# JiuTongBro/MultiView_Inpaint

Hardware: AMD Instinct MI355X
Metric: Mpix/s fwd+bwd @1.5M Gauss 1080p (higher is better)
Workload: dtype f32; 1 GPU; rasterizer-with-depth fwd+bwd, one 1920x1080 view per GPU per step, N=1500000 Gaussians, sh_degree 3 (BASELINE.json configs[2] size, SURVEY.md §8d scene); gaussians=1500000, visible=1312313, num_rendered_D=14779663, tiles=8160, tile_list_max=2266, parallelism=views x1

## Files before the change

### include/mvi_raster.h

```cpp
#ifndef MVI_RASTER_H
#define MVI_RASTER_H

#include <stddef.h>
#include <stdint.h>

#ifdef __cplusplus
extern "C" {
#endif

#define MVI_OK 0
#define MVI_EINVAL (-1)
#define MVI_EHIP (-2)
#define MVI_ENOMEM (-3)

#define MVI_TILE 16

typedef struct mvi_raster_settings {
    int32_t image_height;
    int32_t image_width;
    float tanfovx;
    float tanfovy;
    float scale_modifier;
    int32_t sh_degree;
    int32_t prefiltered;
    const float* bg;
    const float* viewmatrix;
    const float* projmatrix;
    const float* campos;
} mvi_raster_settings;

size_t mvi_raster_geom_bytes(int32_t P);
size_t mvi_raster_image_bytes(int32_t image_width, int32_t image_height);
size_t mvi_raster_binning_bytes(int64_t num_rendered, int32_t image_width, int32_t image_height);

int mvi_raster_forward_geom(const mvi_raster_settings* s, int32_t P, int32_t M,
                            const float* means3D, const float* shs, const float* colors_precomp,
                            const float* opacities, const float* scales, const float* rotations,
                            const float* cov3D_precomp, void* geom, size_t geom_bytes,
                            int32_t* radii, int64_t* num_rendered_host, void* stream);

int mvi_raster_forward_render(const mvi_raster_settings* s, int32_t P, int64_t num_rendered,
                              const int32_t* radii, void* geom, size_t geom_bytes, void* binning, size_t binning_bytes,
                              void* image, size_t image_bytes, float* out_color, float* out_depth,
                              void* stream);
int mvi_raster_forward_render_prepare(const mvi_raster_settings* s, int32_t P, int64_t num_rendered,
                                      const int32_t* radii, void* geom, size_t geom_bytes, void* binning,
                                      size_t binning_bytes, void* image, size_t image_bytes, float* out_color,
                                      float* out_depth, float* grad_rows_scratch, void* stream);

int mvi_raster_backward(const mvi_raster_settings* s, int32_t P, int32_t M, int64_t num_rendered,
                        const float* means3D, const float* shs, const float* colors_precomp,
                        const float* scales, const float* rotations, const float* cov3D_precomp,
                        const int32_t* radii, const void* geom, const void* binning,
                        const void* image, const float* dL_dout_color, float* dL_dmeans3D,
                        float* dL_dmeans2D, float* dL_dopacity, float* dL_dshs, float* dL_dcolors,
                        float* dL_dscales, float* dL_drotations, float* dL_dcov3D,
                        float* grad_rows_scratch, int32_t grad_rows_prezeroed, void* stream);

int mvi_raster_forward_geom_raw(const mvi_raster_settings* s, int32_t P, int32_t M, const float* xyz,
                                const float* features_dc, const float* features_rest, const float* raw_opacity,
                                const float* raw_scaling, const float* raw_rotation, void* geom, size_t geom_bytes,
                                int32_t* radii, int64_t* num_rendered_host, void* stream);
int mvi_raster_backward_raw(const mvi_raster_settings* s, int32_t P, int32_t M, int64_t num_rendered, const float* xyz,
                            const float* features_dc, const float* features_rest, const float* raw_opacity,
                            const float* raw_scaling, const float* raw_rotation, const int32_t* radii, const void* geom,
                            const void* binning, const void* image, const float* dL_dout_color, float* dL_dxyz,
                            float* dL_dmeans2D, float* dL_draw_opacity, float* dL_dfeatures_dc, float* dL_dfeatures_rest,
                            float* dL_draw_scaling, float* dL_draw_rotation, float* grad_rows_scratch, 
                            int32_t grad_rows_prezeroed, void* stream);
int mvi_raster_backward_raw_factor(const mvi_raster_settings* s, int32_t P, int32_t M, int64_t num_rendered, const float* xyz,
                                   const float* features_dc, const float* features_rest, const float* raw_opacity,
                                   const float* raw_scaling, const float* raw_rotation, const int32_t* radii, const void* geom,
                                   const void* binning, const void* image, const float* dL_dout_color, float* dL_dxyz,
                                   float* dL_dmeans2D, float* dL_draw_opacity, float* dL_dsh_color_factor,
                                   float* dL_draw_scaling, float* dL_draw_rotation, float* grad_rows_scratch,
                                   int32_t grad_rows_prezeroed, void* stream);

int mvi_raster_sh_backward_views(int32_t P, int32_t M, int32_t sh_degree, int32_t n_views, const float* means3D,
                                 const float* campos, int64_t campos_stride, const float* dL_dcolors,
                                 int64_t colors_view_stride, float* dL_dshs, void* stream);

int mvi_raster_mark_visible(int32_t P, const float* means3D, const float* viewmatrix,
                            const float* projmatrix, uint8_t* visible, void* stream);

int mvi_raster_backward_render(const mvi_raster_settings* s, int32_t P, int64_t num_rendered, const int32_t* radii,
                               const void* geom, const void* binning, const void* image, const float* dL_dout_color,
                               float* grad_rows_scratch, float* dL_dcolor_factor, int32_t sh_input,
                               int32_t grad_rows_prezeroed, void* stream);
int mvi_raster_backward_geom(const mvi_raster_settings* s, int32_t P, int32_t M, const float* means3D, const float* shs,
                             const float* colors_precomp, const float* scales, const float* rotations,
                             const float* cov3D_precomp, const int32_t* radii, const void* geom,
                             const float* grad_rows_scratch, float* dL_dmeans3D, float* dL_dmeans2D, float* dL_dopacity,
                             float* dL_dshs, float* dL_dcolors, float* dL_dscales, float* dL_drotations, float* dL_dcov3D,
                             void* stream);

int mvi_raster_backward_geom_range(const mvi_raster_settings* s, int32_t P, int32_t M, int32_t first, int32_t count,
                                   const float* means3D, const float* shs, const float* colors_precomp, const float* scales,
                                   const float* rotations, const float* cov3D_precomp, const int32_t* radii, const void* geom,
                                   const float* grad_rows_scratch, float* dL_dmeans3D, float* dL_dmeans2D, float* dL_dopacity,
                                   float* dL_dshs, float* dL_dcolors, float* dL_dscales, float* dL_drotations, float* dL_dcov3D,
                                   void* stream);

typedef struct mvi_raster_views {
    const float* depths;
    const float* means2D;
    const float* cov3D_a;
    const float* cov3D_b;
    const float* conic_opacity;
    const float* rgbd;
    const uint32_t* tiles_touched;
    const uint8_t* clamped;
    const void* tile_ids_sorted;
    const uint32_t* point_list;
    const uint32_t* ranges;
    const float* final_T;
    const uint32_t* n_contrib;
    int32_t tile_id_bytes;
    const uint8_t* grad_support;
} mvi_raster_views;
int mvi_raster_get_views(int32_t P, int64_t num_rendered, int32_t image_width, int32_t image_height,
                         const void* geom, const void* binning, const void* image,
                         mvi_raster_views* out);

#define MVI_RASTER_NSTAGES 8
int mvi_raster_timing_enable(int enable);
int mvi_raster_timing_enable_stages(uint32_t stage_mask);
int mvi_raster_timing_read(float* ms_sum_host, int32_t* calls_host);
const char* mvi_raster_stage_name(int stage);

int mvi_raster_color_mode(int deferred);
int mvi_raster_resolve_colors(const mvi_raster_settings* s, int32_t P, void* geom, size_t geom_bytes, void* stream);

int mvi_raster_binning_version(int version);
int mvi_raster_backward_mode(int dense);
int mvi_raster_dev_stamps(int pass, void* device_buffer);

const char* mvi_raster_last_error(void);
const char* mvi_version(void);

#ifdef __cplusplus
}
#endif
#endif
```

### multiview_inpaint_amd/_lib.py

```python
import ctypes as C
import os
import re

_HERE = os.path.dirname(os.path.abspath(__file__))
LIB_PATH = os.environ.get("MVI_HIP_LIB") or os.path.join(_HERE, "csrc", "libmvi_hip.so")
LIB_OVERRIDDEN = bool(os.environ.get("MVI_HIP_LIB"))
if LIB_OVERRIDDEN:
    import sys as _sys
    _sys.stderr.write(f"[mvi] MVI_HIP_LIB is set: every kernel comes from {LIB_PATH}, not from the in-tree build\n")
INCLUDE_DIR = os.path.normpath(os.path.join(_HERE, "..", "include"))


class RasterSettings(C.Structure):
    _fields_ = [
        ("image_height", C.c_int32), ("image_width", C.c_int32),
        ("tanfovx", C.c_float), ("tanfovy", C.c_float), ("scale_modifier", C.c_float),
        ("sh_degree", C.c_int32), ("prefiltered", C.c_int32),
        ("bg", C.c_void_p), ("viewmatrix", C.c_void_p), ("projmatrix", C.c_void_p), ("campos", C.c_void_p),
    ]


class RasterViews(C.Structure):
    _fields_ = [(n, C.c_void_p) for n in (
        "depths", "means2D", "cov3D_a", "cov3D_b", "conic_opacity", "rgbd", "tiles_touched", "clamped",
        "tile_ids_sorted", "point_list", "ranges", "final_T", "n_contrib")] + [("tile_id_bytes", C.c_int32),
                                                                                   ("grad_support", C.c_void_p)]


class AdamGroup(C.Structure):
    _fields_ = [("param", C.c_void_p), ("grad", C.c_void_p), ("exp_avg", C.c_void_p), ("exp_avg_sq", C.c_void_p),
                ("n", C.c_int64), ("lr", C.c_float)]


class CompactTensor(C.Structure):
    _fields_ = [("in_", C.c_void_p), ("out", C.c_void_p), ("width", C.c_int32), ("packed_stride", C.c_int32)]


def declared_symbols():
    names = []
    for fn in sorted(os.listdir(INCLUDE_DIR)):
        if fn.endswith(".h"):
            src = open(os.path.join(INCLUDE_DIR, fn)).read()
            src = re.sub(r"/\*.*?\*/", "", src, flags=re.S)
            names += re.findall(r"\b(mvi_[a-z0-9_]+)\s*\(", src)
    return sorted(set(names))


def raster_source_digest():
    import hashlib
    h = hashlib.sha1()
    d = os.path.join(_HERE, "csrc")
    for fn in sorted(os.listdir(d)):
        if fn.startswith("raster_") and fn.endswith((".hip", ".h")):
            h.update(fn.encode())
            h.update(open(os.path.join(d, fn), "rb").read())
    return h.hexdigest()[:16]


_lib = None


def lib():
    global _lib
    if _lib is not None:
        return _lib
    if not os.path.exists(LIB_PATH):
        raise RuntimeError(
            f"{LIB_PATH} is missing: the HIP extension is not built. Run `python -m multiview_inpaint_amd.build` "
            "(hipcc --offload-arch=gfx950). There is no CPU or PyTorch fallback for this path.")
    L = C.CDLL(LIB_PATH)
    missing = [s for s in declared_symbols() if not hasattr(L, s)]
    if missing:
        raise RuntimeError(f"{LIB_PATH} does not export {missing}; rebuild it")
    vp, i32, i64, sz = C.c_void_p, C.c_int32, C.c_int64, C.c_size_t
    L.mvi_raster_last_error.restype = C.c_char_p
    L.mvi_version.restype = C.c_char_p
    L.mvi_raster_geom_bytes.restype = sz
    L.mvi_raster_geom_bytes.argtypes = [i32]
    L.mvi_raster_image_bytes.restype = sz
    L.mvi_raster_image_bytes.argtypes = [i32, i32]
    L.mvi_raster_binning_bytes.restype = sz
    L.mvi_raster_binning_bytes.argtypes = [i64, i32, i32]
    L.mvi_raster_forward_geom.restype = C.c_int
    L.mvi_raster_forward_geom.argtypes = [C.POINTER(RasterSettings), i32, i32] + [vp] * 7 + [vp, sz, vp, C.POINTER(i64), vp]
    L.mvi_raster_forward_render.restype = C.c_int
    L.mvi_raster_forward_render.argtypes = [C.POINTER(RasterSettings), i32, i64, vp, vp, sz, vp, sz, vp, sz, vp, vp, vp]
    L.mvi_raster_forward_render_prepare.restype = C.c_int
    L.mvi_raster_forward_render_prepare.argtypes = [C.POINTER(RasterSettings), i32, i64, vp, vp, sz, vp, sz, vp, sz, vp, vp, vp, vp]
    L.mvi_raster_backward.restype = C.c_int
    L.mvi_raster_backward.argtypes = [C.POINTER(RasterSettings), i32, i32, i64] + [vp] * 20 + [i32, vp]
    L.mvi_raster_backward_render.restype = C.c_int
    L.mvi_raster_backward_render.argtypes = [C.POINTER(RasterSettings), i32, i64] + [vp] * 7 + [i32, i32, vp]
    L.mvi_raster_backward_geom.restype = C.c_int
    L.mvi_raster_backward_geom.argtypes = [C.POINTER(RasterSettings), i32, i32] + [vp] * 18
    L.mvi_raster_backward_geom_range.restype = C.c_int
    L.mvi_raster_backward_geom_range.argtypes = [C.POINTER(RasterSettings), i32, i32, i32, i32] + [vp] * 18
    L.mvi_raster_forward_geom_raw.restype = C.c_int
    L.mvi_raster_forward_geom_raw.argtypes = [C.POINTER(RasterSettings), i32, i32] + [vp] * 6 + [vp, sz, vp, C.POINTER(i64), vp]
    L.mvi_raster_backward_raw.restype = C.c_int
    L.mvi_raster_backward_raw.argtypes = [C.POINTER(RasterSettings), i32, i32, i64] + [vp] * 19 + [i32, vp]
    L.mvi_raster_backward_raw_factor.restype = C.c_int
    L.mvi_raster_backward_raw_factor.argtypes = [C.POINTER(RasterSettings), i32, i32, i64] + [vp] * 18 + [i32, vp]
    L.mvi_raster_sh_backward_views.restype = C.c_int
    L.mvi_raster_sh_backward_views.argtypes = [i32, i32, i32, i32, vp, vp, i64, vp, i64, vp, vp]
    L.mvi_raster_mark_visible.restype = C.c_int
    L.mvi_raster_mark_visible.argtypes = [i32, vp, vp, vp, vp, vp]
    L.mvi_raster_get_views.restype = C.c_int
    L.mvi_raster_get_views.argtypes = [i32, i64, i32, i32, vp, vp, vp, C.POINTER(RasterViews)]
    L.mvi_raster_timing_enable.restype = C.c_int
    L.mvi_raster_timing_enable.argtypes = [C.c_int]
    L.mvi_raster_timing_enable_stages.restype = C.c_int
    L.mvi_raster_timing_enable_stages.argtypes = [C.c_uint32]
    L.mvi_raster_timing_read.restype = C.c_int
    L.mvi_raster_timing_read.argtypes = [C.POINTER(C.c_float), C.POINTER(C.c_int32)]
    L.mvi_raster_stage_name.restype = C.c_char_p
    L.mvi_raster_stage_name.argtypes = [C.c_int]
    L.mvi_raster_binning_version.restype = C.c_int
    L.mvi_raster_binning_version.argtypes = [C.c_int]
    L.mvi_raster_backward_mode.restype = C.c_int
    L.mvi_raster_backward_mode.argtypes = [C.c_int]
    L.mvi_raster_color_mode.restype = C.c_int
    L.mvi_raster_color_mode.argtypes = [C.c_int]
    L.mvi_raster_resolve_colors.restype = C.c_int
    L.mvi_raster_resolve_colors.argtypes = [C.POINTER(RasterSettings), i32, vp, sz, vp]
    L.mvi_raster_dev_stamps.restype = C.c_int
    L.mvi_raster_dev_stamps.argtypes = [C.c_int, vp]
    _bind_unet_ops(L)
    _bind_train_ops(L)
    _bind_box_region(L)
    _lib = L
    return L


def _bind_unet_ops(L):
    try:
        from . import _unet_ops_bind
    except ImportError:
        return
    _unet_ops_bind.bind(L)


def _bind_train_ops(L):
    vp, i32, sz, f32 = C.c_void_p, C.c_int32, C.c_size_t, C.c_float
    L.mvi_photometric_loss_workspace_bytes.restype = sz
    L.mvi_photometric_loss_workspace_bytes.argtypes = [i32, i32]
    L.mvi_photometric_loss.restype = C.c_int
    L.mvi_photometric_loss.argtypes = [vp, vp, vp, i32, i32, f32, f32, vp, vp, vp, sz, vp]
    L.mvi_photometric_loss_stats.restype = C.c_int
    L.mvi_photometric_loss_stats.argtypes = [vp, vp, vp, i32, i32, vp, vp, sz, vp]
    L.mvi_photometric_loss_grad2.restype = C.c_int
    L.mvi_photometric_loss_grad2.argtypes = [vp, vp, vp, i32, i32, vp, vp, vp, sz, vp]
    L.mvi_train_last_error.restype = C.c_char_p
    L.mvi_knn3_mean_dist2.restype = C.c_int
    L.mvi_knn3_mean_dist2.argtypes = [vp, i32, vp, vp]
    L.mvi_adam_step.restype = C.c_int
    L.mvi_adam_step.argtypes = [C.POINTER(AdamGroup), i32, C.c_double, C.c_double, C.c_double, i32, vp]
    L.mvi_compact_workspace_bytes.restype = sz
    L.mvi_compact_workspace_bytes.argtypes = [i32]
    L.mvi_compact_plan.restype = C.c_int
    L.mvi_compact_plan.argtypes = [vp, i32, vp, sz, vp, vp]
    L.mvi_compact_gather.restype = C.c_int
    L.mvi_compact_gather.argtypes = [C.POINTER(CompactTensor), i32, i32, C.c_uint32, vp, vp]
    L.mvi_support_pack_bits.restype = C.c_int
    L.mvi_support_pack_bits.argtypes = [vp, i32, vp, vp]
    L.mvi_support_union_bits.restype = C.c_int
    L.mvi_support_union_bits.argtypes = [vp, i32, i32, vp, vp]
    for f in (L.mvi_compact_gather_window, L.mvi_compact_scatter_window):
        f.restype = C.c_int
        f.argtypes = [C.POINTER(CompactTensor), i32, i32, vp, C.c_uint32, C.c_uint32, vp, vp]
    L.mvi_gaussian_activations.restype = C.c_int
    L.mvi_gaussian_activations.argtypes = [i32, i32] + [vp] * 10
    L.mvi_gaussian_activations_backward.restype = C.c_int
    L.mvi_gaussian_activations_backward.argtypes = [i32, i32] + [vp] * 13


def _bind_box_region(L):
    vp, i32, i64 = C.c_void_p, C.c_int32, C.c_int64
    L.mvi_box_region_last_error.restype = C.c_char_p
    L.mvi_mesh_intersect.restype = C.c_int
    L.mvi_mesh_intersect.argtypes = [vp, vp, i64, vp, i32, vp, vp, vp, vp, vp]
    L.mvi_mesh_points_inside.restype = C.c_int
    L.mvi_mesh_points_inside.argtypes = [vp, i64, vp, i32, vp, vp]
    L.mvi_mesh_view_masks.restype = C.c_int
    L.mvi_mesh_view_masks.argtypes = [vp, vp, vp, i32, i32, i32, vp, i32, vp, vp, vp, vp, vp, vp]


def check(rc, what):
    if rc != 0:
        msg = lib().mvi_raster_last_error().decode(errors="replace")
        if rc == -1:
            raise Exception(msg)
        raise RuntimeError(f"{what} failed ({rc}): {msg}")
```

### multiview_inpaint_amd/csrc/raster_api.hip

```cpp
#include <cstdio>
#include <cstdlib>
#include <cstring>

#include "raster_common.h"

namespace mvi {
int launch_scan_block_sums(GeomView g, int P, unsigned long long* total_host_devptr, hipStream_t st);
int launch_zero_fill(void* p, size_t bytes, hipStream_t st);
int launch_binning_level1(const Frame& f, GeomView g, hipStream_t st);
}

static thread_local char g_err[512] = "";
static int g_dense_backward = [] { const char* e = getenv("MVI_RASTER_DENSE_BACKWARD"); return (e && e[0] == '1') ? 1 : 0; }();
static int g_defer_colors = [] { const char* e = getenv("MVI_RASTER_EAGER_COLORS"); return (e && e[0] == '1') ? 0 : 1; }();
#include <mutex>
namespace {
struct SegmentHint { const void* geom; int32_t P; int64_t segments; uint64_t stamp; };
constexpr int kSegmentHints = 64;
SegmentHint g_seg_hints[kSegmentHints] = {};
uint64_t g_seg_clock = 0;
std::mutex g_seg_mutex;
void remember_segments(const void* geom, int32_t P, int64_t segments) {
    std::lock_guard<std::mutex> lock(g_seg_mutex);
    int slot = 0;
    for (int i = 0; i < kSegmentHints; ++i) {
        if (g_seg_hints[i].geom == geom) { slot = i; break; }
        if (g_seg_hints[i].stamp < g_seg_hints[slot].stamp) slot = i;
    }
    g_seg_hints[slot] = {geom, P, segments, ++g_seg_clock};
}
int64_t recall_segments(const void* geom, int32_t P) {
    std::lock_guard<std::mutex> lock(g_seg_mutex);
    for (int i = 0; i < kSegmentHints; ++i)
        if (g_seg_hints[i].geom == geom && g_seg_hints[i].stamp) return g_seg_hints[i].P == P ? g_seg_hints[i].segments : 0;
    return 0;
}
}

#include <vector>
namespace {
struct Rec { int stage; hipEvent_t a, b; };
uint32_t g_timing_mask = 0;
std::vector<Rec> g_recs;
std::vector<hipEvent_t> g_pool;
hipEvent_t g_open[MVI_RASTER_NSTAGES];
hipEvent_t get_event() {
    if (!g_pool.empty()) { hipEvent_t e = g_pool.back(); g_pool.pop_back(); return e; }
    hipEvent_t e; (void)hipEventCreate(&e); return e;
}
}
namespace mvi {
void stage_begin(int stage, hipStream_t st) {
    if (!((g_timing_mask >> stage) & 1u)) return;
    g_open[stage] = get_event();
    (void)hipEventRecord(g_open[stage], st);
}
void stage_end(int stage, hipStream_t st) {
    if (!((g_timing_mask >> stage) & 1u)) return;
    hipEvent_t b = get_event();
    (void)hipEventRecord(b, st);
    g_recs.push_back({stage, g_open[stage], b});
}
}

static int fail(int code, const char* fmt, const char* a = "", long long b = 0, long long c = 0) {
    snprintf(g_err, sizeof(g_err), fmt, a, b, c);
    return code;
}
static int hip_fail(const char* where, hipError_t e) {
    snprintf(g_err, sizeof(g_err), "%s: %s", where, hipGetErrorString(e));
    return MVI_EHIP;
}

static int make_frame(const mvi_raster_settings* s, int P, int M, mvi::Frame& f) {
    if (!s) return fail(MVI_EINVAL, "settings is NULL%s");
    if (s->image_width < 0 || s->image_height < 0 || P < 0)
        return fail(MVI_EINVAL, "negative size%s (P=%lld, W=%lld)", "", P, s->image_width);
    if (s->sh_degree < 0 || s->sh_degree > 3) return fail(MVI_EINVAL, "sh_degree must be 0..3%s (got %lld)", "", s->sh_degree);
    if (!s->bg || !s->viewmatrix || !s->projmatrix || !s->campos)
        return fail(MVI_EINVAL, "bg/viewmatrix/projmatrix/campos must be device pointers%s");
    f.P = P; f.M = M; f.deg = s->sh_degree; f.W = s->image_width; f.H = s->image_height;
    f.gx = (f.W + mvi::kTile - 1) / mvi::kTile;
    f.gy = (f.H + mvi::kTile - 1) / mvi::kTile;
    f.tanfovx = s->tanfovx; f.tanfovy = s->tanfovy;
    f.fx = (float)f.W / (2.0f * s->tanfovx);
    f.fy = (float)f.H / (2.0f * s->tanfovy);
    f.scale_modifier = s->scale_modifier;
    f.view = s->viewmatrix; f.proj = s->projmatrix; f.campos = s->campos; f.bg = s->bg;
    f.bin_v2 = mvi::binning_v2_ok(f.gx, f.gy) ? 1 : 0;
    f.defer_colors = g_defer_colors;
    return MVI_OK;
}

extern "C" {

const char* mvi_raster_last_error(void) { return g_err; }

int mvi_raster_timing_enable(int enable) { g_timing_mask = enable ? (1u << MVI_RASTER_NSTAGES) - 1u : 0u; return MVI_OK; }
int mvi_raster_timing_enable_stages(uint32_t stage_mask) { g_timing_mask = stage_mask & ((1u << MVI_RASTER_NSTAGES) - 1u); return MVI_OK; }
int mvi_raster_timing_read(float* ms_sum, int32_t* calls) {
    if (!ms_sum || !calls) return fail(MVI_EINVAL, "NULL timing outputs%s");
    for (auto& r : g_recs) {
        hipError_t e = hipEventSynchronize(r.b);
        if (e != hipSuccess) return hip_fail("timing sync", e);
        float ms = 0.f;
        (void)hipEventElapsedTime(&ms, r.a, r.b);
        ms_sum[r.stage] += ms;
        calls[r.stage] += 1;
        g_pool.push_back(r.a);
        g_pool.push_back(r.b);
    }
    g_recs.clear();
    return MVI_OK;
}
const char* mvi_raster_stage_name(int i) {
    static const char* n[MVI_RASTER_NSTAGES] = {"preprocess_forward", "scan_block_sums", "duplicate_keys", "radix_sort",
                                                "tile_ranges", "render_forward", "render_backward", "preprocess_backward"};
    return (i >= 0 && i < MVI_RASTER_NSTAGES) ? n[i] : "";
}
int mvi_raster_dev_stamps(int pass, void* device_buffer) { mvi::set_dev_stamps(pass, device_buffer); return MVI_OK; }
int mvi_raster_backward_mode(int dense) {
    const int old = g_dense_backward;
    if (dense == 0 || dense == 1) g_dense_backward = dense;
    return old;
}
int mvi_raster_binning_version(int version) { return mvi::set_binning_version(version); }
int mvi_raster_color_mode(int deferred) {
    const int old = g_defer_colors;
    if (deferred == 0 || deferred == 1) g_defer_colors = deferred;
    return old;
}
int mvi_raster_resolve_colors(const mvi_raster_settings* s, int32_t P, void* geom, size_t geom_bytes, void* stream) {
    mvi::Frame f;
    if (int rc = make_frame(s, P, 0, f)) return rc;
    if (P == 0) return MVI_OK;
    if (!geom) return fail(MVI_EINVAL, "geom is NULL%s");
    mvi::GeomView g = mvi::carve_geom(geom, P);
    if (geom_bytes < g.bytes) return fail(MVI_ENOMEM, "geom scratch too small%s", "");
    if (mvi::launch_resolve_colors(f, g, (hipStream_t)stream)) return hip_fail("resolve_colors", hipGetLastError());
    return MVI_OK;
}
const char* mvi_version(void) { return "multiview_inpaint_amd 0.1.0 (gfx950)"; }

size_t mvi_raster_geom_bytes(int32_t P) { return mvi::carve_geom(nullptr, P).bytes; }
size_t mvi_raster_image_bytes(int32_t W, int32_t H) { return mvi::carve_image(nullptr, W, H).bytes; }
size_t mvi_raster_binning_bytes(int64_t D, int32_t W, int32_t H) { return mvi::carve_binning(nullptr, D, W, H).bytes; }

static int forward_geom_impl(const mvi_raster_settings* s, mvi::Frame& f, int32_t P, int32_t M, const float* means3D,
                             const float* shs, const float* colors_precomp, const float* opacities,
                             const float* scales, const float* rotations, const float* cov3D_precomp,
                             void* geom, size_t geom_bytes, int32_t* radii, int64_t* num_rendered_host,
                             void* stream);

int mvi_raster_forward_geom(const mvi_raster_settings* s, int32_t P, int32_t M, const float* means3D,
                            const float* shs, const float* colors_precomp, const float* opacities,
                            const float* scales, const float* rotations, const float* cov3D_precomp,
                            void* geom, size_t geom_bytes, int32_t* radii, int64_t* num_rendered_host,
                            void* stream) {
    mvi::Frame f;
    if (int rc = make_frame(s, P, M, f)) return rc;
    return forward_geom_impl(s, f, P, M, means3D, shs, colors_precomp, opacities, scales, rotations, cov3D_precomp, geom,
                             geom_bytes, radii, num_rendered_host, stream);
}

int mvi_raster_forward_geom_raw(const mvi_raster_settings* s, int32_t P, int32_t M, const float* xyz,
                                const float* features_dc, const float* features_rest, const float* raw_opacity,
                                const float* raw_scaling, const float* raw_rotation, void* geom, size_t geom_bytes,
                                int32_t* radii, int64_t* num_rendered_host, void* stream) {
    mvi::Frame f;
    if (int rc = make_frame(s, P, M, f)) return rc;
    if (P > 0 && (!features_dc || (M > 1 && !features_rest) || !raw_scaling || !raw_rotation))
        return fail(MVI_EINVAL, "NULL raw parameter pointer%s");
    f.raw = 1;
    f.shs_rest = features_rest;
    return forward_geom_impl(s, f, P, M, xyz, features_dc, nullptr, raw_opacity, raw_scaling, raw_rotation, nullptr, geom,
                             geom_bytes, radii, num_rendered_host, stream);
}

static int forward_geom_impl(const mvi_raster_settings* s, mvi::Frame& f, int32_t P, int32_t M, const float* means3D,
                             const float* shs, const float* colors_precomp, const float* opacities,
                             const float* scales, const float* rotations, const float* cov3D_precomp,
                             void* geom, size_t geom_bytes, int32_t* radii, int64_t* num_rendered_host,
                             void* stream) {
    if (!num_rendered_host) return fail(MVI_EINVAL, "num_rendered_host is NULL%s");
    *num_rendered_host = 0;
    if (P == 0) return MVI_OK;
    if ((shs == nullptr) == (colors_precomp == nullptr))
        return fail(MVI_EINVAL, "Please provide excatly one of either SHs or precomputed colors!%s");
    if (((scales == nullptr) || (rotations == nullptr)) == (cov3D_precomp == nullptr))
        return fail(MVI_EINVAL, "Please provide exactly one of either scale/rotation pair or precomputed 3D covariance!%s");
    if (!means3D || !opacities || !geom || !radii) return fail(MVI_EINVAL, "NULL means3D/opacities/geom/radii%s");
    if (shs && M < (s->sh_degree + 1) * (s->sh_degree + 1))
        return fail(MVI_EINVAL, "shs holds %s%lld coefficients per channel, sh_degree needs %lld", "", M,
                    (s->sh_degree + 1) * (s->sh_degree + 1));
    mvi::GeomView g = mvi::carve_geom(geom, P);
    if (geom_bytes < g.bytes) return fail(MVI_ENOMEM, "geom scratch too small%s: %lld < %lld", "", (long long)geom_bytes, (long long)g.bytes);
    hipStream_t st = (hipStream_t)stream;
    {
        mvi::StageTimer tm(mvi::kStPreFwd, st);
        if (mvi::launch_preprocess_forward(f, means3D, shs, colors_precomp, opacities, scales, rotations,
                                           cov3D_precomp, g, radii, st))
            return hip_fail("preprocess_forward", hipGetLastError());
    }
    struct Readback { unsigned long long* host = nullptr; unsigned long long* dev = nullptr; hipEvent_t ev = nullptr; };
    constexpr int kMaxDevices = 64;
    static thread_local Readback readbacks[kMaxDevices];
    hipError_t e;
    int device = -1;
    if ((e = hipGetDevice(&device)) != hipSuccess) return hip_fail("hipGetDevice", e);
    if (device < 0 || device >= kMaxDevices) return fail(MVI_EINVAL, "device index out of range%s: %lld", "", (long long)device);
    Readback& rb = readbacks[device];
    if (!rb.host) {
        unsigned long long* h = nullptr;
        if ((e = hipHostMalloc((void**)&h, 2 * sizeof(unsigned long long), hipHostMallocMapped | hipHostMallocPortable)) != hipSuccess) return hip_fail("hipHostMalloc", e);
        if ((e = hipHostGetDevicePointer((void**)&rb.dev, h, 0)) != hipSuccess) { (void)hipHostFree(h); return hip_fail("hipHostGetDevicePointer", e); }
        if ((e = hipEventCreateWithFlags(&rb.ev, hipEventDisableTiming)) != hipSuccess) { (void)hipHostFree(h); return hip_fail("hipEventCreate", e); }
        rb.host = h;
    }
    unsigned long long* const pinned = rb.host;
    unsigned long long* const pinned_dev = rb.dev;
    const hipEvent_t ev = rb.ev;
    {
        mvi::StageTimer tm(mvi::kStScan, st);
        if (f.bin_v2 ? mvi::launch_binning2_totals(g, P, pinned_dev, st) : mvi::launch_scan_block_sums(g, P, pinned_dev, st))
            return hip_fail("scan_block_sums", hipGetLastError());
    }
    if ((e = hipEventRecord(ev, st)) != hipSuccess) return hip_fail("event record", e);
    if (f.bin_v2 ? mvi::launch_binning2_level1(f, g, st) : mvi::launch_binning_level1(f, g, st))
        return hip_fail("binning level 1", hipGetLastError());
    e = hipEventSynchronize(ev);
    if (e != hipSuccess) return hip_fail("forward_geom sync", e);
    const unsigned long long total = *pinned;
    if (total > 0xFFFFFFFFull)
        return fail(MVI_EINVAL, "num_rendered exceeds the 32-bit pair offsets%s: %lld pairs", "", (long long)total);
    *num_rendered_host = (int64_t)total;
    if (f.bin_v2) remember_segments(geom, P, (int64_t)pinned[1]);
    return MVI_OK;
}

static int forward_render_impl(const mvi_raster_settings* s, int32_t P, int64_t D, const int32_t* radii,
                               void* geom, size_t geom_bytes, void* binning, size_t binning_bytes, void* image,
                               size_t image_bytes, float* out_color, float* out_depth, float* grad_rows_to_zero, void* stream) {
    mvi::Frame f;
    if (int rc = make_frame(s, P, 0, f)) return rc;
    if (!image || !out_color || !out_depth) return fail(MVI_EINVAL, "NULL image/out_color/out_depth%s");
    if (D < 0 || D > 0xFFFFFFFFll) return fail(MVI_EINVAL, "num_rendered out of range%s: %lld", "", D);
    if (D > 0 && (!geom || !binning || !radii)) return fail(MVI_EINVAL, "NULL geom/binning/radii with num_rendered > 0%s");
    mvi::GeomView g = mvi::carve_geom(geom, P);
    mvi::ImageView im = mvi::carve_image(image, f.W, f.H);
    mvi::BinningView b = mvi::carve_binning(binning, D, f.W, f.H);
    if (image_bytes < im.bytes) return fail(MVI_ENOMEM, "image scratch too small%s: %lld < %lld", "", (long long)image_bytes, (long long)im.bytes);
    if (D > 0 && binning_bytes < b.bytes) return fail(MVI_ENOMEM, "binning scratch too small%s: %lld < %lld", "", (long long)binning_bytes, (long long)b.bytes);
    if (D > 0 && geom_bytes < g.bytes) return fail(MVI_ENOMEM, "geom scratch too small%s", "");
    hipStream_t st = (hipStream_t)stream;
    const int64_t segments = recall_segments(geom, P);
    if (f.bin_v2 ? mvi::launch_binning2(f, g, b, im, D, segments, st) : mvi::launch_binning(f, g, radii, b, im, D, st))
        return hip_fail("binning", hipGetLastError());
    {
        mvi::StageTimer tm(mvi::kStRenderFwd, st);
        if (mvi::launch_render_forward(f, g, b, im, D, out_color, out_depth, st, grad_rows_to_zero))
            return hip_fail("render_forward", hipGetLastError());
    }
    return MVI_OK;
}

int mvi_raster_forward_render(const mvi_raster_settings* s, int32_t P, int64_t D, const int32_t* radii,
                              void* geom, size_t geom_bytes, void* binning, size_t binning_bytes, void* image,
                              size_t image_bytes, float* out_color, float* out_depth, void* stream) {
    return forward_render_impl(s, P, D, radii, geom, geom_bytes, binning, binning_bytes, image, image_bytes, out_color, out_depth,
                               nullptr, stream);
}

int mvi_raster_forward_render_prepare(const mvi_raster_settings* s, int32_t P, int64_t D, const int32_t* radii,
                                      void* geom, size_t geom_bytes, void* binning, size_t binning_bytes, void* image,
                                      size_t image_bytes, float* out_color, float* out_depth, float* grad_rows_scratch,
                                      void* stream) {
    return forward_render_impl(s, P, D, radii, geom, geom_bytes, binning, binning_bytes, image, image_bytes, out_color, out_depth,
                               grad_rows_scratch, stream);
}

static int backward_render_impl(mvi::Frame& f, int32_t P, int64_t D, const int32_t* radii, const void* geom, const void* binning,
                                const void* image, const float* dL_dout_color, float* grad_rows, float* dL_dcolor_factor,
                                int sh_input, int rows_prezeroed, void* stream, const mvi::ZeroRegions* zero_outputs = nullptr);
static int backward_impl(mvi::Frame& f, int32_t P, int64_t D, const float* means3D, const float* shs,
                         const float* colors_precomp, const float* scales, const float* rotations,
                         const float* cov3D_precomp, const int32_t* radii, const void* geom, const void* binning,
                         const void* image, const float* dL_dout_color, float* dL_dmeans3D, float* dL_dmeans2D,
                         float* dL_dopacity, float* dL_dshs, float* dL_dcolors, float* dL_dscales, float* dL_drotations,
                         float* dL_dcov3D, float* dL_dconic_scratch, void* stream, mvi::RawBackwardExtra rawx);

int mvi_raster_backward(const mvi_raster_settings* s, int32_t P, int32_t M, int64_t D, const float* means3D,
                        const float* shs, const float* colors_precomp, const float* scales,
                        const float* rotations, const float* cov3D_precomp, const int32_t* radii,
                        const void* geom, const void* binning, const void* image,
                        const float* dL_dout_color, float* dL_dmeans3D, float* dL_dmeans2D,
                        float* dL_dopacity, float* dL_dshs, float* dL_dcolors, float* dL_dscales,
                        float* dL_drotations, float* dL_dcov3D, float* dL_dconic_scratch, int32_t grad_rows_prezeroed,
                        void* stream) {
    mvi::Frame f;
    if (int rc = make_frame(s, P, M, f)) return rc;
    mvi::RawBackwardExtra rawx;
    rawx.rows_prezeroed = grad_rows_prezeroed;
    return backward_impl(f, P, D, means3D, shs, colors_precomp, scales, rotations, cov3D_precomp, radii, geom, binning, image,
                         dL_dout_color, dL_dmeans3D, dL_dmeans2D, dL_dopacity, dL_dshs, dL_dcolors, dL_dscales, dL_drotations,
                         dL_dcov3D, dL_dconic_scratch, stream, rawx);
}

int mvi_raster_backward_raw(const mvi_raster_settings* s, int32_t P, int32_t M, int64_t D, const float* xyz,
                            const float* features_dc, const float* features_rest, const float* raw_opacity,
                            const float* raw_scaling, const float* raw_rotation, const int32_t* radii, const void* geom,
                            const void* binning, const void* image, const float* dL_dout_color, float* dL_dxyz,
                            float* dL_dmeans2D, float* dL_draw_opacity, float* dL_dfeatures_dc, float* dL_dfeatures_rest,
                            float* dL_draw_scaling, float* dL_draw_rotation, float* grad_rows_scratch,
                            int32_t grad_rows_prezeroed, void* stream) {
    mvi::Frame f;
    if (int rc = make_frame(s, P, M, f)) return rc;
    if (P > 0 && (!features_dc || (M > 1 && (!features_rest || !dL_dfeatures_rest)) || !raw_opacity || !dL_dfeatures_dc))
        return fail(MVI_EINVAL, "NULL raw parameter / gradient pointer%s");
    f.raw = 1;
    f.shs_rest = features_rest;
    mvi::RawBackwardExtra rawx;
    rawx.raw_opacity = raw_opacity;
    rawx.dL_dshs_rest = dL_dfeatures_rest;
    rawx.rows_prezeroed = grad_rows_prezeroed;
    return backward_impl(f, P, D, xyz, features_dc, nullptr, raw_scaling, raw_rotation, nullptr, radii, geom, binning, image,
                         dL_dout_color, dL_dxyz, dL_dmeans2D, dL_draw_opacity, dL_dfeatures_dc, nullptr, dL_draw_scaling,
                         dL_draw_rotation, nullptr, grad_rows_scratch, stream, rawx);
}

int mvi_raster_backward_raw_factor(const mvi_raster_settings* s, int32_t P, int32_t M, int64_t D, const float* xyz,
                                   const float* features_dc, const float* features_rest, const float* raw_opacity,
                                   const float* raw_scaling, const float* raw_rotation, const int32_t* radii, const void* geom,
                                   const void* binning, const void* image, const float* dL_dout_color, float* dL_dxyz,
                                   float* dL_dmeans2D, float* dL_draw_opacity, float* dL_dsh_color_factor, float* dL_draw_scaling,
                                   float* dL_draw_rotation, float* grad_rows_scratch, int32_t grad_rows_prezeroed, void* stream) {
    mvi::Frame f;
    if (int rc = make_frame(s, P, M, f)) return rc;
    if (P > 0 && (!features_dc || (M > 1 && !features_rest) || !raw_opacity || !dL_dsh_color_factor))
        return fail(MVI_EINVAL, "NULL raw parameter / colour factor pointer%s");
    f.raw = 1;
    f.shs_rest = features_rest;
    mvi::RawBackwardExtra rawx;
    rawx.raw_opacity = raw_opacity;
    rawx.dL_dshs_rest = nullptr;
    rawx.rows_prezeroed = grad_rows_prezeroed;
    return backward_impl(f, P, D, xyz, features_dc, nullptr, raw_scaling, raw_rotation, nullptr, radii, geom, binning, image,
                         dL_dout_color, dL_dxyz, dL_dmeans2D, dL_draw_opacity, nullptr, dL_dsh_color_factor, dL_draw_scaling,
                         dL_draw_rotation, nullptr, grad_rows_scratch, stream, rawx);
}

static int backward_impl(mvi::Frame& f, int32_t P, int64_t D, const float* means3D, const float* shs,
                         const float* colors_precomp, const float* scales, const float* rotations,
                         const float* cov3D_precomp, const int32_t* radii, const void* geom, const void* binning,
                         const void* image, const float* dL_dout_color, float* dL_dmeans3D, float* dL_dmeans2D,
                         float* dL_dopacity, float* dL_dshs, float* dL_dcolors, float* dL_dscales, float* dL_drotations,
                         float* dL_dcov3D, float* dL_dconic_scratch, void* stream, mvi::RawBackwardExtra rawx) {
    if (P == 0) return MVI_OK;
    if ((shs == nullptr) == (colors_precomp == nullptr))
        return fail(MVI_EINVAL, "Please provide excatly one of either SHs or precomputed colors!%s");
    if (((scales == nullptr) || (rotations == nullptr)) == (cov3D_precomp == nullptr))
        return fail(MVI_EINVAL, "Please provide exactly one of either scale/rotation pair or precomputed 3D covariance!%s");
    if (!means3D || !radii || !geom || !image || !dL_dout_color || !dL_dmeans3D || !dL_dmeans2D || !dL_dopacity ||
        !dL_dconic_scratch)
        return fail(MVI_EINVAL, "NULL required pointer in backward%s");
    if (shs && !dL_dshs && !dL_dcolors)
        return fail(MVI_EINVAL, "dL_dshs and dL_dcolors are both NULL but shs was a forward input%s");
    if (colors_precomp && !dL_dcolors) return fail(MVI_EINVAL, "dL_dcolors is NULL but colors_precomp was a forward input%s");
    if (cov3D_precomp ? !dL_dcov3D : (!dL_dscales || !dL_drotations))
        return fail(MVI_EINVAL, "missing covariance gradient output%s");
    if (D > 0 && !binning) return fail(MVI_EINVAL, "NULL binning with num_rendered > 0%s");
    const bool dense_bwd = g_dense_backward != 0;
    mvi::GeomView g = mvi::carve_geom(const_cast<void*>(geom), P);
    hipStream_t st = (hipStream_t)stream;
    if (!dense_bwd) {
        mvi::ZeroRegions z;
        const size_t n = (size_t)P, Mz = (size_t)f.M;
        z.add(dL_dmeans3D, 3 * n);
        z.add(dL_dmeans2D, 3 * n);
        z.add(dL_dopacity, n);
        if (dL_dcolors) z.add(dL_dcolors, 3 * n);
        if (shs && dL_dshs) z.add(dL_dshs, f.raw ? 3 * n : 3 * Mz * n);
        if (f.raw && rawx.dL_dshs_rest && Mz > 1) z.add(rawx.dL_dshs_rest, (3 * Mz - 3) * n);
        if (cov3D_precomp) z.add(dL_dcov3D, 6 * n);
        else { z.add(dL_dscales, 3 * n); z.add(dL_drotations, 4 * n); }
        if (z.overflow) return fail(MVI_EINVAL, "more gradient outputs than the render backward can zero on the side%s (kMaxZero)");
        if (int rc = backward_render_impl(f, P, D, radii, geom, binning, image, dL_dout_color, dL_dconic_scratch, nullptr, 0,
                                          rawx.rows_prezeroed, stream, &z)) return rc;
        mvi::StageTimer tm(mvi::kStPreBwd, st);
        if (mvi::launch_preprocess_backward_sparse(f, means3D, shs, scales, rotations, cov3D_precomp, g, dL_dconic_scratch,
                                                   dL_dmeans3D, dL_dmeans2D, dL_dopacity, dL_dcolors, dL_dshs, dL_dcov3D,
                                                   dL_dscales, dL_drotations, st, rawx))
            return hip_fail("preprocess_backward (sparse)", hipGetLastError());
        return MVI_OK;
    }
    if (int rc = backward_render_impl(f, P, D, radii, geom, binning, image, dL_dout_color, dL_dconic_scratch, nullptr, 0,
                                      rawx.rows_prezeroed, stream)) return rc;
    mvi::StageTimer tm(mvi::kStPreBwd, st);
    if (mvi::launch_preprocess_backward(f, means3D, shs, scales, rotations, cov3D_precomp, radii, g, dL_dconic_scratch,
                                        dL_dmeans3D, dL_dmeans2D, dL_dopacity, dL_dcolors,
                                        dL_dshs, dL_dcov3D, dL_dscales, dL_drotations, st, rawx))
        return hip_fail("preprocess_backward", hipGetLastError());
    return MVI_OK;
}

static int backward_render_impl(mvi::Frame& f, int32_t P, int64_t D, const int32_t* radii, const void* geom, const void* binning,
                                const void* image, const float* dL_dout_color, float* grad_rows, float* dL_dcolor_factor,
                                int sh_input, int rows_prezeroed, void* stream, const mvi::ZeroRegions* zero_outputs) {
    if (P == 0) return MVI_OK;
    if (!radii || !geom || !image || !dL_dout_color || !grad_rows) return fail(MVI_EINVAL, "NULL required pointer in backward%s");
    if (D > 0 && !binning) return fail(MVI_EINVAL, "NULL binning with num_rendered > 0%s");
    mvi::GeomView g = mvi::carve_geom(const_cast<void*>(geom), P);
    mvi::ImageView im = mvi::carve_image(const_cast<void*>(image), f.W, f.H);
    mvi::BinningView b = mvi::carve_binning(const_cast<void*>(binning), D, f.W, f.H);
    hipStream_t st = (hipStream_t)stream;
    if (!rows_prezeroed) {
        mvi::ZeroRegions z;
        z.add(grad_rows, (size_t)mvi::kGradRow * (size_t)P);
        z.add(g.touched, ((size_t)P + 15) / 16 * 4);
        z.add(g.touched_count, 1);
        if (mvi::launch_zero_regions(z, st)) return hip_fail("zero grad rows", hipGetLastError());
    }
    {
        mvi::StageTimer tm(mvi::kStRenderBwd, st);
        if (mvi::launch_render_backward(f, g, b, im, D, dL_dout_color, grad_rows, st, zero_outputs))
            return hip_fail("render_backward", hipGetLastError());
    }
    if (dL_dcolor_factor && mvi::launch_color_factors(P, radii, grad_rows, sh_input ? g.clamped : nullptr, dL_dcolor_factor, st))
        return hip_fail("color_factors", hipGetLastError());
    return MVI_OK;
}

int mvi_raster_backward_render(const mvi_raster_settings* s, int32_t P, int64_t D, const int32_t* radii, const void* geom,
                               const void* binning, const void* image, const float* dL_dout_color, float* grad_rows_scratch,
                               float* dL_dcolor_factor, int32_t sh_input, int32_t grad_rows_prezeroed, void* stream) {
    mvi::Frame f;
    if (int rc = make_frame(s, P, 0, f)) return rc;
    return backward_render_impl(f, P, D, radii, geom, binning, image, dL_dout_color, grad_rows_scratch, dL_dcolor_factor,
                                sh_input, grad_rows_prezeroed, stream);
}

static int backward_geom_range_impl(const mvi_raster_settings* s, int32_t P, int32_t M, int32_t first, int32_t count,
                                    const float* means3D, const float* shs, const float* colors_precomp, const float* scales,
                                    const float* rotations, const float* cov3D_precomp, const int32_t* radii, const void* geom,
                                    const float* grad_rows_scratch, float* dL_dmeans3D, float* dL_dmeans2D, float* dL_dopacity,
                                    float* dL_dshs, float* dL_dcolors, float* dL_dscales, float* dL_drotations, float* dL_dcov3D,
                                    void* stream) {
    mvi::Frame f;
    if (int rc = make_frame(s, P, M, f)) return rc;
    if (first < 0 || count < 0 || (int64_t)first + count > P || (first % 64) != 0)
        return fail(MVI_EINVAL, "backward range out of bounds or not 64-aligned%s: first %lld count %lld", "", (long long)first, (long long)count);
    if (P == 0 || count == 0) return MVI_OK;
    if ((shs == nullptr) == (colors_precomp == nullptr))
        return fail(MVI_EINVAL, "Please provide excatly one of either SHs or precomputed colors!%s");
    if (((scales == nullptr) || (rotations == nullptr)) == (cov3D_precomp == nullptr))
        return fail(MVI_EINVAL, "Please provide exactly one of either scale/rotation pair or precomputed 3D covariance!%s");
    if (!means3D || !radii || !geom || !grad_rows_scratch || !dL_dmeans3D || !dL_dmeans2D || !dL_dopacity)
        return fail(MVI_EINVAL, "NULL required pointer in backward%s");
    if (shs && !dL_dshs && !dL_dcolors)
        return fail(MVI_EINVAL, "dL_dshs and dL_dcolors are both NULL but shs was a forward input%s");
    if (colors_precomp && !dL_dcolors) return fail(MVI_EINVAL, "dL_dcolors is NULL but colors_precomp was a forward input%s");
    if (cov3D_precomp ? !dL_dcov3D : (!dL_dscales || !dL_drotations))
        return fail(MVI_EINVAL, "missing covariance gradient output%s");
    mvi::GeomView g = mvi::carve_geom(const_cast<void*>(geom), P);
    const size_t o = (size_t)first;
    g.depths += o; g.xy += o; g.cov_a += o; g.cov_b += o; g.conic_opacity += o; g.rgbd += o; g.tiles_touched += o; g.rect += o;
    g.clamped += o;
    auto at = [o](auto* p, size_t w) { return p ? p + o * w : p; };
    f.P = count;
    hipStream_t st = (hipStream_t)stream;
    mvi::StageTimer tm(mvi::kStPreBwd, st);
    if (mvi::launch_preprocess_backward(f, at(means3D, 3), at(shs, 3 * (size_t)M), at(scales, 3), at(rotations, 4), at(cov3D_precomp, 6),
                                        at(radii, 1), g, at(grad_rows_scratch, 16), at(dL_dmeans3D, 3), at(dL_dmeans2D, 3),
                                        at(dL_dopacity, 1), at(dL_dcolors, 3), at(dL_dshs, 3 * (size_t)M), at(dL_dcov3D, 6),
                                        at(dL_dscales, 3), at(dL_drotations, 4), st, mvi::RawBackwardExtra()))
        return hip_fail("preprocess_backward", hipGetLastError());
    return MVI_OK;
}

int mvi_raster_backward_geom(const mvi_raster_settings* s, int32_t P, int32_t M, const float* means3D, const float* shs,
                             const float* colors_precomp, const float* scales, const float* rotations,
                             const float* cov3D_precomp, const int32_t* radii, const void* geom,
                             const float* grad_rows_scratch, float* dL_dmeans3D, float* dL_dmeans2D, float* dL_dopacity,
                             float* dL_dshs, float* dL_dcolors, float* dL_dscales, float* dL_drotations, float* dL_dcov3D,
                             void* stream) {
    return backward_geom_range_impl(s, P, M, 0, P, means3D, shs, colors_precomp, scales, rotations, cov3D_precomp, radii, geom,
                                    grad_rows_scratch, dL_dmeans3D, dL_dmeans2D, dL_dopacity, dL_dshs, dL_dcolors, dL_dscales,
                                    dL_drotations, dL_dcov3D, stream);
}

int mvi_raster_backward_geom_range(const mvi_raster_settings* s, int32_t P, int32_t M, int32_t first, int32_t count,
                                   const float* means3D, const float* shs, const float* colors_precomp, const float* scales,
                                   const float* rotations, const float* cov3D_precomp, const int32_t* radii, const void* geom,
                                   const float* grad_rows_scratch, float* dL_dmeans3D, float* dL_dmeans2D, float* dL_dopacity,
                                   float* dL_dshs, float* dL_dcolors, float* dL_dscales, float* dL_drotations, float* dL_dcov3D,
                                   void* stream) {
    return backward_geom_range_impl(s, P, M, first, count, means3D, shs, colors_precomp, scales, rotations, cov3D_precomp, radii,
                                    geom, grad_rows_scratch, dL_dmeans3D, dL_dmeans2D, dL_dopacity, dL_dshs, dL_dcolors, dL_dscales,
                                    dL_drotations, dL_dcov3D, stream);
}

int mvi_raster_sh_backward_views(int32_t P, int32_t M, int32_t sh_degree, int32_t n_views, const float* means3D,
                                 const float* campos, int64_t campos_stride, const float* dL_dcolors,
                                 int64_t colors_view_stride, float* dL_dshs, void* stream) {
    if (P < 0 || M < 1 || M > 16 || sh_degree < 0 || (sh_degree + 1) * (sh_degree + 1) > M || n_views < 1)
        return fail(MVI_EINVAL, "bad shape for sh_backward_views (need 1 <= (deg+1)^2 <= M <= 16, n_views >= 1)%s");
    if (P == 0) return MVI_OK;
    if (!means3D || !campos || !dL_dcolors || !dL_dshs) return fail(MVI_EINVAL, "NULL pointer in sh_backward_views%s");
    if (campos_stride < 3 || colors_view_stride < 3 * (int64_t)P)
        return fail(MVI_EINVAL, "sh_backward_views: campos_stride must be >= 3 and colors_view_stride >= 3 P%s");
    if (mvi::launch_sh_backward_views(P, M, sh_degree, n_views, means3D, campos, campos_stride, dL_dcolors,
                                      colors_view_stride, dL_dshs, (hipStream_t)stream))
        return hip_fail("sh_backward_views", hipGetLastError());
    return MVI_OK;
}

int mvi_raster_mark_visible(int32_t P, const float* means3D, const float* viewmatrix, const float* projmatrix,
                            uint8_t* visible, void* stream) {
    if (P < 0 || (P > 0 && (!means3D || !viewmatrix || !visible))) return fail(MVI_EINVAL, "bad arguments to mark_visible%s");
    if (mvi::launch_mark_visible(P, means3D, viewmatrix, visible, (hipStream_t)stream)) return hip_fail("mark_visible", hipGetLastError());
    return MVI_OK;
}

int mvi_raster_get_views(int32_t P, int64_t D, int32_t W, int32_t H, const void* geom, const void* binning,
                         const void* image, mvi_raster_views* out) {
    if (!out) return fail(MVI_EINVAL, "views is NULL%s");
    memset(out, 0, sizeof(*out));
    if (geom) {
        mvi::GeomView g = mvi::carve_geom(const_cast<void*>(geom), P);
        out->depths = g.depths; out->means2D = reinterpret_cast<const float*>(g.xy);
        out->cov3D_a = reinterpret_cast<const float*>(g.cov_a); out->cov3D_b = reinterpret_cast<const float*>(g.cov_b);
        out->conic_opacity = reinterpret_cast<const float*>(g.conic_opacity); out->rgbd = reinterpret_cast<const float*>(g.rgbd);
        out->tiles_touched = g.tiles_touched; out->clamped = g.clamped;
        out->grad_support = g.touched;
    }
    if (binning) {
        mvi::BinningView b = mvi::carve_binning(const_cast<void*>(binning), D, W, H);
        int fin = b.passes & 1;
        out->tile_ids_sorted = b.keys[fin]; out->point_list = b.vals[fin];
        out->tile_id_bytes = b.key_bytes;
    }
    if (image) {
        mvi::ImageView im = mvi::carve_image(const_cast<void*>(image), W, H);
        out->ranges = im.ranges; out->final_T = im.final_T; out->n_contrib = im.n_contrib;
    }
    return MVI_OK;
}

}
```

### multiview_inpaint_amd/csrc/raster_binning2.hip

```cpp
#include <cstdlib>

#include "raster_common.h"

namespace mvi {

static int g_binning_version = [] { const char* e = getenv("MVI_BINNING_LEGACY"); return (e && e[0] == '1') ? 1 : 2; }();
bool binning_v2_enabled() { return g_binning_version == 2; }
int set_binning_version(int v) {
    const int old = g_binning_version;
    if (v == 1 || v == 2) g_binning_version = v;
    return old;
}

__device__ __forceinline__ uint32_t block_excl_scan256(uint32_t v, int tid, uint32_t* s_w4, uint32_t* total) {
    const int lane = tid & 63, wave = tid >> 6;
    uint32_t inc = v;
#pragma unroll
    for (int o = 1; o < 64; o <<= 1) {
        uint32_t t = __shfl_up(inc, o);
        if (lane >= o) inc += t;
    }
    if (wave < 4 && lane == 63) s_w4[wave] = inc;
    __syncthreads();
    uint32_t off = 0;
#pragma unroll
    for (int w = 0; w < 3; ++w) if (w < wave) off += s_w4[w];
    if (total) *total = s_w4[0] + s_w4[1] + s_w4[2] + s_w4[3];
    __syncthreads();
    return off + inc - v;
}

__global__ __launch_bounds__(1024) void totals2_kernel(const uint32_t* __restrict__ pair_sums,
                                                       const uint32_t* __restrict__ seg_sums, int n,
                                                       uint32_t* __restrict__ super0, int super_words,
                                                       uint32_t* __restrict__ arrivals,
                                                       unsigned long long* __restrict__ totals_host) {
    __shared__ unsigned long long s_wave[2][16];
    const int tid = threadIdx.x;
    for (int i = tid; i < super_words; i += 1024) super0[i] = 0u;
    if (tid == 0) *arrivals = 0u;
    unsigned long long a = 0, b = 0;
    const int n4 = n >> 2;
    const uint4* p4 = reinterpret_cast<const uint4*>(pair_sums);
    const uint4* s4 = reinterpret_cast<const uint4*>(seg_sums);
#pragma unroll 4
    for (int i = tid; i < n4; i += 1024) {
        const uint4 u = p4[i], v = s4[i];
        a += (unsigned long long)u.x + u.y + u.z + u.w;
        b += (unsigned long long)v.x + v.y + v.z + v.w;
    }
    for (int i = 4 * n4 + tid; i < n; i += 1024) { a += pair_sums[i]; b += seg_sums[i]; }
#pragma unroll
    for (int d = 32; d >= 1; d >>= 1) { a += __shfl_xor(a, d); b += __shfl_xor(b, d); }
    if ((tid & 63) == 0) { s_wave[0][tid >> 6] = a; s_wave[1][tid >> 6] = b; }
    __syncthreads();
    if (tid < 2) {
        unsigned long long t = 0;
#pragma unroll
        for (int w = 0; w < 16; ++w) t += s_wave[tid][w];
        if (totals_host) __hip_atomic_store(totals_host + tid, t, __ATOMIC_RELEASE, __HIP_MEMORY_SCOPE_SYSTEM);
    }
}
int launch_binning2_totals(GeomView g, int P, unsigned long long* totals_host_devptr, hipStream_t st) {
    const int npre = (P + kPB - 1) / kPB;
    hipLaunchKernelGGL(totals2_kernel, dim3(1), dim3(1024), 0, st, g.block_sums, g.seg_sums, npre, g.ds_super[0],
                       256 * g.nsuper, g.arrivals, totals_host_devptr);
    return hipGetLastError() == hipSuccess ? 0 : MVI_EHIP;
}

__device__ __forceinline__ void lds_wave_sync() {
    asm volatile("s_waitcnt lgkmcnt(0)" ::: "memory");
    __builtin_amdgcn_wave_barrier();
}

__global__ __launch_bounds__(kDsThreads) void depth_count_kernel(const uint32_t* __restrict__ keys, int P, int shift,
                                                                 uint32_t* __restrict__ table,
                                                                 uint32_t* __restrict__ super) {
    static_assert(kDsThreads == 256, "thread = digit");
    __shared__ uint32_t s_h[256];
    const int tid = threadIdx.x;
    s_h[tid] = 0;
    __syncthreads();
    const int base = blockIdx.x * kDsTile;
    uint4 k4[kDsItems / 4];
#pragma unroll
    for (int it = 0; it < kDsItems / 4; ++it) {
        const int i0 = base + (it * kDsThreads + tid) * 4;
        k4[it] = i0 < P ? *reinterpret_cast<const uint4*>(keys + i0) : make_uint4(0u, 0u, 0u, 0u);
    }
#pragma unroll
    for (int it = 0; it < kDsItems / 4; ++it) {
        const int i0 = base + (it * kDsThreads + tid) * 4;
        if (i0 < P) {
            const uint32_t k[4] = {k4[it].x, k4[it].y, k4[it].z, k4[it].w};
            uint32_t d_prev = (k[0] >> shift) & 255u, run = 1;
#pragma unroll
            for (int j = 1; j < 4; ++j) {
                const uint32_t d = (k[j] >> shift) & 255u;
                if (i0 + j < P) {
                    if (d == d_prev) ++run;
                    else { atomicAdd(&s_h[d_prev], run); d_prev = d; run = 1; }
                }
            }
            atomicAdd(&s_h[d_prev], run);
        }
    }
    __syncthreads();
    const uint32_t c = s_h[tid];
    table[(size_t)blockIdx.x * 256 + tid] = c;
    if (c) atomicAdd(&super[(size_t)(blockIdx.x / kDsSuper) * 256 + tid], c);
}

template <int PASS>
__global__ __launch_bounds__(kDsThreads) void depth_scatter_kernel(
    const uint32_t* __restrict__ keys_in, const uint32_t* __restrict__ vals_in, uint32_t* __restrict__ keys_out,
    uint32_t* __restrict__ vals_out, int P, const uint32_t* __restrict__ table, const uint32_t* __restrict__ super,
    int nsuper, uint32_t* __restrict__ super_next, const uint2* __restrict__ rect, uint2* __restrict__ rect_sorted) {
    constexpr int kW = kDsThreads / 64;
    constexpr int shift = 8 * PASS;
    __shared__ uint32_t s_wave_hist[kW][256];
    __shared__ unsigned long long s_match[kW][256];
    __shared__ uint32_t s_digit_base[256];
    __shared__ uint32_t s_local_start[256];
    __shared__ uint32_t s_red[4][2][256];
    __shared__ uint32_t s_w4[4];
    __shared__ uint32_t s_key[kDsTile];
    __shared__ uint32_t s_val[kDsTile];
    const int tid = threadIdx.x, lane = tid & 63, wave = tid >> 6;
#pragma unroll
    for (int i = tid; i < kW * 256; i += kDsThreads) { (&s_wave_hist[0][0])[i] = 0; (&s_match[0][0])[i] = 0ull; }

    const int tile0 = blockIdx.x * kDsTile;
    const int base = tile0 + wave * (kDsItems * 64);
    uint32_t key[kDsItems], val[kDsItems];
#pragma unroll
    for (int it = 0; it < kDsItems; ++it) {
        const int idx = base + it * 64 + lane;
        const bool valid = idx < P;
        key[it] = valid ? keys_in[idx] : 0u;
        val[it] = PASS == 0 ? (uint32_t)idx : (valid ? vals_in[idx] : 0u);
    }
    uint2 rc[PASS == 3 ? kDsItems : 1];
    if (PASS == 3) {
#pragma unroll
        for (int it = 0; it < kDsItems; ++it)
            rc[it] = (base + it * 64 + lane) < P ? rect[val[it]] : make_uint2(0u, 0u);
    }
    {
        const int dq = tid & 63, rg = tid >> 6;
        const int grp = (int)blockIdx.x / kDsSuper;
        uint4 all = make_uint4(0u, 0u, 0u, 0u), bef = make_uint4(0u, 0u, 0u, 0u);
#pragma unroll 4
        for (int j = rg; j < nsuper; j += 4) {
            const uint4 c = *reinterpret_cast<const uint4*>(super + (size_t)j * 256 + 4 * dq);
            all.x += c.x; all.y += c.y; all.z += c.z; all.w += c.w;
            if (j < grp) { bef.x += c.x; bef.y += c.y; bef.z += c.z; bef.w += c.w; }
        }
#pragma unroll
        for (int j = rg; j < kDsSuper - 1; j += 4) {
            const int t = grp * kDsSuper + j;
            if (t < (int)blockIdx.x) {
                const uint4 c = *reinterpret_cast<const uint4*>(table + (size_t)t * 256 + 4 * dq);
                bef.x += c.x; bef.y += c.y; bef.z += c.z; bef.w += c.w;
            }
        }
        *reinterpret_cast<uint4*>(&s_red[rg][0][4 * dq]) = all;
        *reinterpret_cast<uint4*>(&s_red[rg][1][4 * dq]) = bef;
        if (super_next && blockIdx.x == 0)
            for (int i = tid; i < 256 * nsuper; i += kDsThreads) super_next[i] = 0u;
    }
    __syncthreads();
    const uint32_t all = s_red[0][0][tid] + s_red[1][0][tid] + s_red[2][0][tid] + s_red[3][0][tid];
    const uint32_t before = s_red[0][1][tid] + s_red[1][1][tid] + s_red[2][1][tid] + s_red[3][1][tid];
    uint32_t dinc = all;
#pragma unroll
    for (int o = 1; o < 64; o <<= 1) {
        uint32_t t = __shfl_up(dinc, o);
        if (lane >= o) dinc += t;
    }
    if (lane == 63) s_w4[wave] = dinc;

    uint32_t rank[kDsItems], dig[kDsItems];
    const unsigned long long bit = 1ull << lane, lt = bit - 1ull;
    unsigned long long* const mk = s_match[wave];
    uint32_t* const cnt = s_wave_hist[wave];
#pragma unroll
    for (int it = 0; it < kDsItems; ++it) {
        const bool valid = (base + it * 64 + lane) < P;
        const uint32_t d = (key[it] >> shift) & 255u;
        dig[it] = valid ? d : 0xFFFFFFFFu;
        if (valid) atomicOr(&mk[d], bit);
        lds_wave_sync();
        const unsigned long long m = valid ? mk[d] : 0ull;
        const uint32_t prev = valid ? cnt[d] : 0u;
        lds_wave_sync();
        if (valid && (m >> lane) == 1ull) { cnt[d] = prev + (uint32_t)__popcll(m); mk[d] = 0ull; }
        rank[it] = prev + (uint32_t)__popcll(m & lt);
    }
    __syncthreads();
    {
        uint32_t wave_off = 0;
        for (int w = 0; w < wave; ++w) wave_off += s_w4[w];
        s_digit_base[tid] = wave_off + dinc - all + before;
    }
    uint32_t tot = 0;
    {
        uint32_t run = 0;
#pragma unroll
        for (int w = 0; w < kW; ++w) {
            const uint32_t c = s_wave_hist[w][tid];
            s_wave_hist[w][tid] = run;
            run += c;
        }
        tot = run;
    }
    uint32_t inc = tot;
#pragma unroll
    for (int o = 1; o < 64; o <<= 1) {
        uint32_t t = __shfl_up(inc, o);
        if (lane >= o) inc += t;
    }
    __syncthreads();
    if (lane == 63) s_w4[wave] = inc;
    __syncthreads();
    {
        uint32_t wave_off = 0;
        for (int w = 0; w < wave; ++w) wave_off += s_w4[w];
        s_local_start[tid] = wave_off + inc - tot;
    }
    __syncthreads();
#pragma unroll
    for (int it = 0; it < kDsItems; ++it) {
        if (dig[it] != 0xFFFFFFFFu) {
            const uint32_t d = dig[it];
            const uint32_t lp = s_local_start[d] + s_wave_hist[wave][d] + rank[it];
            s_key[lp] = key[it];
            s_val[lp] = val[it];
            if (PASS == 3) rect_sorted[s_digit_base[d] + (lp - s_local_start[d])] = rc[it];
        }
    }
    __syncthreads();
    const int count = (P - tile0) < kDsTile ? (P - tile0) : kDsTile;
#pragma unroll
    for (int it = 0; it < kDsItems; ++it) {
        const int lp = it * kDsThreads + tid;
        if (lp < count) {
            const uint32_t k = s_key[lp];
            const uint32_t d = (k >> shift) & 255u;
            const uint32_t dst = s_digit_base[d] + ((uint32_t)lp - s_local_start[d]);
            if (PASS != 3) keys_out[dst] = k;
            vals_out[dst] = s_val[lp];
        }
    }
}

__global__ __launch_bounds__(kExThreads) void column_count_kernel(int P, int gx, const uint2* __restrict__ rect_sorted,
                                                                  uint32_t* __restrict__ col_table, int nblk1) {
    __shared__ uint32_t s_d[257];
    __shared__ uint32_t s_w4[4];
    const int tid = threadIdx.x;
    if (tid <= 256) s_d[tid] = 0;
    const int base = blockIdx.x * kExChunk;
    uint2 rc[kExItems];
#pragma unroll
    for (int k = 0; k < kExItems; ++k) {
        const int i = base + k * kExThreads + tid;
        rc[k] = i < P ? rect_sorted[i] : make_uint2(0u, 0u);
    }
    __syncthreads();
#pragma unroll
    for (int k = 0; k < kExItems; ++k) {
        const uint32_t x0 = rc[k].x & 0xFFFFu, w = rc[k].y & 0xFFFFu, h = rc[k].y >> 16;
        if (w * h) { atomicAdd(&s_d[x0], 1u); atomicSub(&s_d[x0 + w], 1u); }
    }
    __syncthreads();
    const uint32_t v = tid < 256 ? s_d[tid] : 0u;
    const uint32_t ex = block_excl_scan256(v, tid, s_w4, nullptr);
    if (tid < gx) col_table[(size_t)tid * nblk1 + blockIdx.x] = ex + v;
}

__device__ __forceinline__ void build_chunk_table(const uint32_t* col_tot, int gx, int tid, uint32_t* __restrict__ chunk_first,
                                                  uint32_t* __restrict__ col_start, uint32_t* s_w4) {
    const uint32_t v = tid < gx ? __hip_atomic_load(col_tot + tid, __ATOMIC_RELAXED, __HIP_MEMORY_SCOPE_AGENT) : 0u;
    const uint32_t c = tid < gx ? max(1u, (v + (uint32_t)kEx2Chunk - 1u) / (uint32_t)kEx2Chunk) : 0u;
    uint32_t tv, tc;
    const uint32_t ev = block_excl_scan256(v, tid, s_w4, &tv);
    const uint32_t ec = block_excl_scan256(c, tid, s_w4, &tc);
    if (tid < gx) { col_start[tid] = ev; chunk_first[tid] = ec; }
    if (tid == 0) { col_start[gx] = tv; chunk_first[gx] = tc; }
}
__global__ __launch_bounds__(1024) void columns_scan_kernel(uint32_t* __restrict__ table, int stride, int n,
                                                            uint32_t* __restrict__ tot, int gx, uint32_t* __restrict__ arrivals,
                                                            uint32_t* __restrict__ chunk_first,
                                                            uint32_t* __restrict__ col_start) {
    __shared__ uint32_t s_wave[16];
    __shared__ uint32_t s_carry, s_last;
    __shared__ uint32_t s_w4[4];
    uint32_t* row = table + (size_t)blockIdx.x * stride;
    const int tid = threadIdx.x, lane = tid & 63, wave = tid >> 6;
    if (tid == 0) s_carry = 0;
    __syncthreads();
    for (int base = 0; base < n; base += 1024) {
        const int i = base + tid;
        const uint32_t v = i < n ? row[i] : 0u;
        uint32_t inc = v;
#pragma unroll
        for (int o = 1; o < 64; o <<= 1) {
            uint32_t t = __shfl_up(inc, o);
            if (lane >= o) inc += t;
        }
        if (lane == 63) s_wave[wave] = inc;
        __syncthreads();
        uint32_t wave_off = 0;
        for (int w = 0; w < wave; ++w) wave_off += s_wave[w];
        const uint32_t carry = s_carry;
        if (i < n) row[i] = carry + wave_off + inc - v;
        __syncthreads();
        if (tid == 1023) s_carry = carry + wave_off + inc;
        __syncthreads();
    }
    if (tid == 0) {
        __hip_atomic_store(tot + blockIdx.x, s_carry, __ATOMIC_RELAXED, __HIP_MEMORY_SCOPE_AGENT);
        asm volatile("s_waitcnt vmcnt(0)" ::: "memory");
        const uint32_t prev = __hip_atomic_fetch_add(arrivals, 1u, __ATOMIC_RELAXED, __HIP_MEMORY_SCOPE_AGENT);
        s_last = prev == (uint32_t)gridDim.x - 1u;
        if (s_last) __hip_atomic_store(arrivals, 0u, __ATOMIC_RELAXED, __HIP_MEMORY_SCOPE_AGENT);
    }
    __syncthreads();
    if (!s_last) return;
    build_chunk_table(tot, gx, tid, chunk_first, col_start, s_w4);
}
struct Chunk { int x; uint32_t seg0, seg1; bool first; };
__device__ __forceinline__ bool load_chunk(const uint32_t* __restrict__ chunk_first, const uint32_t* __restrict__ col_start,
                                           int gx, int tid, uint32_t* s_first, uint32_t* s_col, Chunk& ck) {
    if (tid <= gx) { s_first[tid] = chunk_first[tid]; s_col[tid] = col_start[tid]; }
    __syncthreads();
    const uint32_t c = blockIdx.x;
    if (c >= s_first[gx]) return false;
    int lo = 0, hi = gx - 1;
    while (lo < hi) {
        const int mid = (lo + hi + 1) >> 1;
        if (s_first[mid] <= c) lo = mid; else hi = mid - 1;
    }
    ck.x = lo;
    ck.first = c == s_first[lo];
    ck.seg0 = s_col[lo] + (c - s_first[lo]) * (uint32_t)kEx2Chunk;
    ck.seg1 = min(ck.seg0 + (uint32_t)kEx2Chunk, s_col[lo + 1]);
    return true;
}

__global__ __launch_bounds__(kExThreads) void row_count_kernel(int gx, int gy, const uint32_t* __restrict__ chunk_first,
                                                               const uint32_t* __restrict__ col_start,
                                                               const uint16_t* __restrict__ seg_yh,
                                                               uint32_t* __restrict__ row_table, int stride) {
    __shared__ uint32_t s_first[257], s_col[257], s_w4[4];
    __shared__ uint32_t s_d[257];
    const int tid = threadIdx.x;
    if (tid <= 256) s_d[tid] = 0;
    Chunk ck;
    if (!load_chunk(chunk_first, col_start, gx, tid, s_first, s_col, ck)) return;
#pragma unroll
    for (int k = 0; k < kEx2Items; ++k) {
        const uint32_t i = ck.seg0 + (uint32_t)(k * kExThreads + tid);
        if (i < ck.seg1) {
            const uint32_t yh = seg_yh[i];
            const uint32_t y0 = yh & 255u, h = (yh >> 8) + 1u;
            atomicAdd(&s_d[y0], 1u);
            atomicSub(&s_d[y0 + h], 1u);
        }
    }
    __syncthreads();
    const uint32_t v = tid < 256 ? s_d[tid] : 0u;
    const uint32_t ex = block_excl_scan256(v, tid, s_w4, nullptr);
    if (tid < gy) row_table[(size_t)tid * stride + blockIdx.x] = ex + v;
}

__global__ __launch_bounds__(1024) void row_scan_kernel(int gx, const uint32_t* __restrict__ chunk_first,
                                                        uint32_t* __restrict__ row_table, int stride,
                                                        uint32_t* __restrict__ row_tot, uint32_t* __restrict__ col_rel) {
    __shared__ uint32_t s_first[257];
    __shared__ uint32_t s_wave[16];
    __shared__ uint32_t s_carry;
    const int tid = threadIdx.x, lane = tid & 63, wave = tid >> 6;
    if (tid <= gx) s_first[tid] = chunk_first[tid];
    if (tid == 0) s_carry = 0;
    __syncthreads();
    const int n = (int)s_first[gx];
    uint32_t* row = row_table + (size_t)blockIdx.x * stride;
    for (int base = 0; base < n; base += 1024) {
        const int i = base + tid;
        const uint32_t v = i < n ? row[i] : 0u;
        uint32_t inc = v;
#pragma unroll
        for (int o = 1; o < 64; o <<= 1) {
            uint32_t t = __shfl_up(inc, o);
            if (lane >= o) inc += t;
        }
        if (lane == 63) s_wave[wave] = inc;
        __syncthreads();
        uint32_t wave_off = 0;
        for (int w = 0; w < wave; ++w) wave_off += s_wave[w];
        const uint32_t carry = s_carry;
        if (i < n) row[i] = carry + wave_off + inc - v;
        __syncthreads();
        if (tid == 1023) s_carry = carry + wave_off + inc;
        __syncthreads();
    }
    __syncthreads();
    uint32_t* cr = col_rel + (size_t)blockIdx.x * (gx + 1);
    if (tid < gx) cr[tid] = __hip_atomic_load(row + s_first[tid], __ATOMIC_RELAXED, __HIP_MEMORY_SCOPE_AGENT);
    if (tid == 0) { cr[gx] = s_carry; row_tot[blockIdx.x] = s_carry; }
}

struct ExpandArgs {
    int n_items;
    int nbins;
    int gx;
    const uint32_t* order;
    const uint2* rect_sorted;
    const uint32_t* chunk_first;
    const uint32_t* col_start;
    const uint32_t* seg_idx_in;
    const uint16_t* seg_yh_in;
    const uint32_t* col_rel;
    uint32_t* ranges;
    const uint32_t* table;
    const uint32_t* tot;
    int stride;
    uint32_t* out_idx;
    uint16_t* out_aux;
    unsigned long long* stamps;
};
static unsigned long long* g_dev_stamps[2] = {nullptr, nullptr};
void set_dev_stamps(int pass, void* buf) { if (pass == 1 || pass == 2) g_dev_stamps[pass - 1] = (unsigned long long*)buf; }
#define MVI_STAMP(i) do { if (A.stamps && tid == 0) A.stamps[(size_t)blk * 8 + (i)] = __builtin_amdgcn_s_memtime(); } while (0)

__device__ __forceinline__ void block_excl_scan512x2(uint32_t a, uint32_t b, int tid, uint32_t (*s_w)[8], uint32_t& ea,
                                                     uint32_t& ta, uint32_t& eb) {
    const int lane = tid & 63, wave = tid >> 6;
    uint32_t ia = a, ib = b;
#pragma unroll
    for (int o = 1; o < 64; o <<= 1) {
        const uint32_t x = __shfl_up(ia, o), y = __shfl_up(ib, o);
        if (lane >= o) { ia += x; ib += y; }
    }
    if (lane == 63) { s_w[0][wave] = ia; s_w[1][wave] = ib; }
    __syncthreads();
    uint32_t oa = 0, ob = 0, t = 0;
#pragma unroll
    for (int w = 0; w < 8; ++w) {
        const uint32_t x = s_w[0][w], y = s_w[1][w];
        if (w < wave) { oa += x; ob += y; }
        t += x;
    }
    ea = oa + ia - a; eb = ob + ib - b; ta = t;
}

template <int PASS, int NB, int ITEMS, int CAP>
__global__ __launch_bounds__(kExThreads) void expand_scatter_kernel(ExpandArgs A) {
    constexpr int kChunk = kExThreads * ITEMS;
    constexpr int kCap = CAP;
    constexpr int kRounds = kChunk / 64;
    constexpr int kStride = NB + 1;
    static_assert(kCap >= 64 * NB, "a round of 64 items (<= 64 * NB entries) always fits the image");
    static_assert(kRounds >= 16, "worker parts <= rounds");
    static_assert(kExThreads == 512, "block_excl_scan512x2");
    __shared__ alignas(16) unsigned long long s_mask[kRounds * kStride + 1];
    __shared__ uint32_t s_pay[kChunk];
    __shared__ uint16_t s_aux[PASS == 1 ? kChunk : 1];
    __shared__ uint32_t s_img[kCap];
    __shared__ uint32_t s_lstart[NB + 1], s_delta[NB];
    __shared__ uint32_t s_rtot[kRounds];
    __shared__ uint32_t s_w[2][8];
    uint32_t* const s_first = s_img;
    uint32_t* const s_col = s_img + 257;
    const int tid = threadIdx.x, lane = tid & 63, wave = tid >> 6;
    const uint32_t blk = blockIdx.x;

    uint32_t item0 = 0, item1 = 0;
    Chunk ck{0, 0u, 0u, false};
    if (PASS == 1) {
        item0 = blk * (uint32_t)kChunk;
        item1 = min(item0 + (uint32_t)kChunk, (uint32_t)A.n_items);
    } else {
        if (!load_chunk(A.chunk_first, A.col_start, A.gx, tid, s_first, s_col, ck)) return;
        item0 = ck.seg0; item1 = ck.seg1;
    }
    MVI_STAMP(0);
    uint32_t ia[ITEMS], in_[ITEMS];
#pragma unroll
    for (int k = 0; k < ITEMS; ++k) {
        const int li = (wave * ITEMS + k) * 64 + lane;
        const uint32_t i = item0 + (uint32_t)li;
        ia[k] = 0; in_[k] = 0;
        uint32_t pay = 0, aux = 0;
        if (i < item1) {
            if (PASS == 1) {
                const uint2 rc = A.rect_sorted[i];
                const uint32_t w = rc.y & 0xFFFFu, h = rc.y >> 16;
                if (w * h) {
                    ia[k] = rc.x & 0xFFFFu; in_[k] = w;
                    pay = A.order[i];
                    aux = (rc.x >> 16) | ((h - 1u) << 8);
                }
            } else {
                const uint32_t yh = A.seg_yh_in[i];
                ia[k] = yh & 255u; in_[k] = (yh >> 8) + 1u;
                pay = A.seg_idx_in[i];
            }
        }
        s_pay[li] = pay;
        if (PASS == 1) s_aux[li] = (uint16_t)aux;
    }
    const int nb = A.nbins;
    const int parts = min(kExThreads / nb, 16);
    const bool worker = tid < parts * nb;
    const int b = worker ? tid / parts : 0, q = worker ? tid % parts : 0;
    const int r_lo = worker ? q * kRounds / parts : 0, r_hi = worker ? (q + 1) * kRounds / parts : 0;
    const bool bin_head = worker && q == 0;
    const uint32_t bin_tot = bin_head ? A.tot[b] : 0u;
    const uint32_t bin_off = bin_head ? A.table[(size_t)b * A.stride + blk] : 0u;
    {
        uint4* m4 = reinterpret_cast<uint4*>(&s_mask[0]);
        for (int i = tid; i < (kRounds * kStride + 1) / 2; i += kExThreads) m4[i] = make_uint4(0u, 0u, 0u, 0u);
        if (tid < kRounds) s_rtot[tid] = 0;
    }
    __syncthreads();
    MVI_STAMP(1);

    const unsigned long long bit = 1ull << lane;
#pragma unroll
    for (int k = 0; k < ITEMS; ++k) {
        unsigned long long* row = s_mask + (wave * ITEMS + k) * kStride;
        for (uint32_t i = 0; i < in_[k]; ++i) atomicOr(&row[ia[k] + i], bit);
    }
    __syncthreads();
    MVI_STAMP(2);

    const unsigned long long* mcol = s_mask + b;
    uint32_t my_base = 0, my_goff = 0;

    int g0 = 0, g1 = kRounds;
    bool first = true, have_rtot = false;
    for (;;) {
        uint32_t cnt = 0;
        for (int r = max(r_lo, g0); r < min(r_hi, g1); ++r) cnt += (uint32_t)__popcll(mcol[r * kStride]);
        uint32_t pos0, total, bin_start;
        block_excl_scan512x2(cnt, first ? bin_tot : 0u, tid, s_w, pos0, total, bin_start);
        if (first) {
            first = false;
            my_base = bin_start + bin_off;
            if (PASS == 2 && ck.first && bin_head) {
                const uint32_t* cr = A.col_rel + (size_t)b * (A.gx + 1);
                const uint32_t c = cr[ck.x + 1] - cr[ck.x];
                uint2* rg = reinterpret_cast<uint2*>(A.ranges) + ((size_t)b * A.gx + ck.x);
                *rg = c ? make_uint2(my_base, my_base + c) : make_uint2(0u, 0u);
            }
            if (total == 0) return;
        }
        MVI_STAMP(3);
        if (total > (uint32_t)kCap) {
            if (!have_rtot) {
                have_rtot = true;
                for (int r = r_lo; r < r_hi; ++r) {
                    const uint32_t c = (uint32_t)__popcll(mcol[r * kStride]);
                    if (c) atomicAdd(&s_rtot[r], c);
                }
            }
            __syncthreads();
            uint32_t acc = 0;
            g1 = g0;
            while (g1 < kRounds && acc + s_rtot[g1] <= (uint32_t)kCap) { acc += s_rtot[g1]; ++g1; }
            continue;
        }
        if (bin_head) {
            s_lstart[b] = pos0;
            s_delta[b] = my_base + my_goff - pos0;
        }
        if (tid == 0) s_lstart[nb] = total;
        MVI_STAMP(4);
        if (cnt) {
            uint32_t pos = pos0;
            const uint32_t hi = (uint32_t)b << 16;
            for (int r = max(r_lo, g0); r < min(r_hi, g1); ++r) {
                const unsigned long long m = mcol[r * kStride];
                uint32_t m0 = (uint32_t)m, m1 = (uint32_t)(m >> 32);
                const uint32_t item_hi = hi | (uint32_t)(r * 64);
                while (m0) {
                    const uint32_t l = (uint32_t)__builtin_ctz(m0);
                    m0 &= m0 - 1u;
                    s_img[pos++] = item_hi | l;
                }
                while (m1) {
                    const uint32_t l = (uint32_t)__builtin_ctz(m1);
                    m1 &= m1 - 1u;
                    s_img[pos++] = item_hi | 32u | l;
                }
            }
        }
        __syncthreads();
        MVI_STAMP(5);
        for (uint32_t p = tid; p < total; p += kExThreads) {
            const uint32_t e = s_img[p];
            const uint32_t eb = e >> 16, item = e & 0xFFFFu;
            const uint32_t dst = p + s_delta[eb];
            A.out_idx[dst] = s_pay[item];
            if (PASS == 1) A.out_aux[dst] = s_aux[item];
            else A.out_aux[dst] = (uint16_t)(eb * (uint32_t)A.gx + (uint32_t)ck.x);
        }
        MVI_STAMP(6);
        if (g1 >= kRounds) break;
        if (bin_head) my_goff += s_lstart[b + 1] - pos0;
        __syncthreads();
        g0 = g1; g1 = kRounds;
    }
}

int launch_binning2_level1(const Frame& f, GeomView g, hipStream_t st) {
    if (f.P <= 0) return 0;
    {
        StageTimer tm(kStSort, st);
#define MVI_DS_PASS(PASS, SRC, DST)                                                                                              \
        hipLaunchKernelGGL(depth_count_kernel, dim3(g.nds), dim3(kDsThreads), 0, st, g.dkeys[SRC], f.P, 8 * PASS, g.ds_table,     \
                           g.ds_super[PASS & 1]);                                                                                 \
        hipLaunchKernelGGL((depth_scatter_kernel<PASS>), dim3(g.nds), dim3(kDsThreads), 0, st, g.dkeys[SRC], g.dvals[SRC],        \
                           g.dkeys[DST], g.dvals[DST], f.P, g.ds_table, g.ds_super[PASS & 1], g.nsuper,                           \
                           PASS < 3 ? g.ds_super[(PASS + 1) & 1] : (uint32_t*)nullptr, g.rect, g.rect_sorted);
        MVI_DS_PASS(0, 0, 1) MVI_DS_PASS(1, 1, 0) MVI_DS_PASS(2, 0, 1) MVI_DS_PASS(3, 1, 0)
#undef MVI_DS_PASS
    }
    StageTimer tm(kStDup, st);
    hipLaunchKernelGGL(column_count_kernel, dim3(g.nblk1), dim3(kExThreads), 0, st, f.P, f.gx, g.rect_sorted, g.col_table,
                       g.nblk1);
    hipLaunchKernelGGL(columns_scan_kernel, dim3(f.gx), dim3(1024), 0, st, g.col_table, g.nblk1, g.nblk1, g.col_tot, f.gx,
                       g.arrivals, g.chunk_first, g.col_start);
    return hipGetLastError() == hipSuccess ? 0 : MVI_EHIP;
}

int launch_binning2(const Frame& f, GeomView g, BinningView b, ImageView im, int64_t D, int64_t segments, hipStream_t st) {
    const size_t tiles = (size_t)f.gx * f.gy;
    if (D <= 0 || f.P <= 0) return launch_zero_fill(im.ranges, 8 * tiles, st);
    const bool wide = f.gx > 128 || f.gy > 128;
    ExpandArgs a1{};
    a1.n_items = f.P; a1.nbins = f.gx; a1.gx = f.gx;
    a1.order = g.dvals[0]; a1.rect_sorted = g.rect_sorted;
    a1.table = g.col_table; a1.tot = g.col_tot; a1.stride = g.nblk1;
    a1.out_idx = b.vals[0]; a1.out_aux = (uint16_t*)b.keys[0];
    a1.stamps = g_dev_stamps[0];
    {
        StageTimer tm(kStDup, st);
        if (wide)
            hipLaunchKernelGGL((expand_scatter_kernel<1, 256, kExItems, 64 * 256>), dim3(g.nblk1), dim3(kExThreads), 0, st, a1);
        else hipLaunchKernelGGL((expand_scatter_kernel<1, 128, kExItems, 64 * 128>), dim3(g.nblk1), dim3(kExThreads), 0, st, a1);
    }
    int nchunk = b.nsort;
    if (segments > 0 && segments <= D) nchunk = (int)min((int64_t)b.nsort, segments / kEx2Chunk + f.gx + 1);
    ExpandArgs a2{};
    a2.nbins = f.gy; a2.gx = f.gx;
    a2.chunk_first = g.chunk_first; a2.col_start = g.col_start;
    a2.seg_idx_in = b.vals[0]; a2.seg_yh_in = (const uint16_t*)b.keys[0];
    a2.col_rel = b.col_rel; a2.ranges = im.ranges;
    a2.table = b.block_hist; a2.tot = b.digit_tot; a2.stride = b.nsort;
    a2.out_idx = b.vals[1]; a2.out_aux = (uint16_t*)b.keys[1];
    a2.stamps = g_dev_stamps[1];
    StageTimer tm(kStSort, st);
    hipLaunchKernelGGL(row_count_kernel, dim3(nchunk), dim3(kExThreads), 0, st, f.gx, f.gy, g.chunk_first, g.col_start,
                       (const uint16_t*)b.keys[0], b.block_hist, b.nsort);
    hipLaunchKernelGGL(row_scan_kernel, dim3(f.gy), dim3(1024), 0, st, f.gx, g.chunk_first, b.block_hist, b.nsort,
                       b.digit_tot, b.col_rel);
    if (f.gy <= kEx2SmallNB)
        hipLaunchKernelGGL((expand_scatter_kernel<2, kEx2SmallNB, kEx2Items, kEx2SmallCap>), dim3(nchunk), dim3(kExThreads), 0,
                           st, a2);
    else if (f.gy <= 128)
        hipLaunchKernelGGL((expand_scatter_kernel<2, 128, kEx2Items, 64 * 128>), dim3(nchunk), dim3(kExThreads), 0, st, a2);
    else hipLaunchKernelGGL((expand_scatter_kernel<2, 256, kEx2Items, 64 * 256>), dim3(nchunk), dim3(kExThreads), 0, st, a2);
    return hipGetLastError() == hipSuccess ? 0 : MVI_EHIP;
}

}
```

### multiview_inpaint_amd/csrc/raster_common.h

```cpp
#pragma once
#include <hip/hip_runtime.h>
#include <stdint.h>
#include <stddef.h>
#include <type_traits>

#include "../../include/mvi_raster.h"

namespace mvi {

constexpr int kTile = MVI_TILE;
constexpr int kBlock = 256;
constexpr int kPB = 64;
constexpr float kNearZ = 0.2f;
constexpr float kLowpass = 0.3f;
constexpr float kFrustumClamp = 1.3f;
constexpr float kLambdaFloor = 0.1f;
constexpr float kAlphaMax = 0.99f;
constexpr float kAlphaMin = 1.0f / 255.0f;
constexpr float kTEps = 0.0001f;
constexpr float kDepthSentinel = 15.0f;

constexpr int kSortItems = 8;
constexpr int kSortWavesP = 4;
constexpr int kSortWavesD = 8;
constexpr int kCountTiles = 4;
__host__ __device__ inline int sort_blocks(int64_t n, int waves) {
    const int tile = 512 * waves;
    int b = (int)((n + tile - 1) / tile);
    return (b + kCountTiles - 1) / kCountTiles * kCountTiles;
}

struct Frame {
    int P, M, deg, W, H, gx, gy;
    float tanfovx, tanfovy, fx, fy, scale_modifier;
    const float* view;
    const float* proj;
    const float* campos;
    const float* bg;
    const float* shs_rest = nullptr;
    int raw = 0;
    int bin_v2 = 0;
    int defer_colors = 0;
};

constexpr int kDsThreads = 256;
constexpr int kDsItems = 8;
constexpr int kDsTile = kDsThreads * kDsItems;
constexpr int kDsSuper = 16;
constexpr int kExThreads = 512;
constexpr int kExItems = 4;
constexpr int kExChunk = kExThreads * kExItems;
constexpr int kEx2Items = 3;
constexpr int kEx2Chunk = kExThreads * kEx2Items;
constexpr int kEx2SmallNB = 80;
constexpr int kEx2SmallCap = 7168;
bool binning_v2_enabled();
void set_dev_stamps(int pass, void* buf);
int set_binning_version(int v);
inline bool binning_v2_ok(int gx, int gy) { return gx <= 256 && gy <= 256 && binning_v2_enabled(); }

struct ColorSource {
    const float* means3D;
    const float* shs;
    const float* shs_rest;
    int32_t M, deg, raw;
    int32_t deferred;
    int32_t vec16;
};

struct GeomView {
    float* depths;
    float2* xy;
    float4* cov_a;
    float2* cov_b;
    float4* conic_opacity;
    float4* rgbd;
    uint32_t* tiles_touched;
    uint2* rect;
    uint8_t* clamped;
    uint8_t* front;
    struct ColorSource* color_src;
    uint32_t* touched_list;
    uint32_t* touched_count;
    uint8_t* touched;
    uint32_t* block_sums;
    uint32_t* block_offsets;
    uint32_t* dkeys[2];
    uint32_t* dvals[2];
    uint32_t* dhist;
    uint32_t* dtot;
    uint32_t* perm_sums;
    uint32_t* perm_offsets;
    uint2* rect_sorted;
    uint32_t* col_table;
    uint32_t* col_tot;
    uint32_t* seg_sums;
    uint32_t* chunk_first;
    uint32_t* col_start;
    uint32_t* arrivals;
    uint32_t* ds_table;
    uint32_t* ds_super[2];
    int nds, nsuper;
    int nblk1;
    int nsortP;
    size_t bytes;
};
struct ImageView {
    uint32_t* ranges;
    float* final_T;
    uint32_t* n_contrib;
    size_t bytes;
};
struct BinningView {
    void* keys[2];
    int key_bytes;
    uint32_t* vals[2];
    uint32_t* block_hist;
    uint32_t* digit_tot;
    int nsort;
    int passes;
    int key_bits;
    int v2;
    uint32_t* col_rel;
    size_t bytes;
};

inline size_t align256(size_t x) { return (x + 255) & ~size_t(255); }

inline GeomView carve_geom(void* base, int P) {
    GeomView g;
    char* p = (char*)base;
    size_t o = 0;
    size_t n = (size_t)(P > 0 ? P : 1);
    int nblk = (int)((n + kBlock - 1) / kBlock);
    auto take = [&](size_t b) { char* r = p ? p + o : nullptr; o += align256(b); return r; };
    g.depths = (float*)take(4 * n);
    g.xy = (float2*)take(8 * n);
    g.cov_a = (float4*)take(16 * n);
    g.cov_b = (float2*)take(8 * n);
    g.conic_opacity = (float4*)take(16 * n);
    g.rgbd = (float4*)take(16 * n);
    g.tiles_touched = (uint32_t*)take(4 * n);
    g.rect = (uint2*)take(8 * n);
    g.clamped = (uint8_t*)take(n);
    g.touched = (uint8_t*)take(n);
    g.touched_list = (uint32_t*)take(4 * n);
    g.touched_count = (uint32_t*)take(4);
    g.front = (uint8_t*)take(n);
    g.color_src = (ColorSource*)take(sizeof(ColorSource));
    const size_t npre = (n + kPB - 1) / kPB;
    g.block_sums = (uint32_t*)take(4 * npre);
    g.block_offsets = (uint32_t*)take(4 * (npre + 1));
    g.nsortP = sort_blocks(n, kSortWavesP);
    for (int i = 0; i < 2; ++i) { g.dkeys[i] = (uint32_t*)take(4 * n); g.dvals[i] = (uint32_t*)take(4 * n); }
    g.dhist = (uint32_t*)take(4 * 256 * (size_t)g.nsortP);
    g.dtot = (uint32_t*)take(4 * 256);
    g.perm_sums = (uint32_t*)take(4 * (size_t)nblk);
    g.perm_offsets = (uint32_t*)take(4 * (size_t)(nblk + 1));
    g.rect_sorted = (uint2*)take(8 * n);
    g.nblk1 = (int)((n + kExChunk - 1) / kExChunk);
    g.col_table = (uint32_t*)take(4 * 256 * (size_t)g.nblk1);
    g.col_tot = (uint32_t*)take(4 * 256);
    g.seg_sums = (uint32_t*)take(4 * npre);
    g.chunk_first = (uint32_t*)take(4 * 257);
    g.col_start = (uint32_t*)take(4 * 257);
    g.arrivals = (uint32_t*)take(4);
    g.nds = (int)((n + kDsTile - 1) / kDsTile);
    g.nsuper = (g.nds + kDsSuper - 1) / kDsSuper;
    g.ds_table = (uint32_t*)take(4 * 256 * (size_t)g.nds);
    g.ds_super[0] = (uint32_t*)take(4 * 256 * (size_t)g.nsuper);
    g.ds_super[1] = (uint32_t*)take(4 * 256 * (size_t)g.nsuper);
    g.bytes = o;
    return g;
}
inline ImageView carve_image(void* base, int W, int H) {
    ImageView v;
    char* p = (char*)base;
    size_t o = 0;
    size_t tiles = (size_t)((W + kTile - 1) / kTile) * ((H + kTile - 1) / kTile);
    size_t px = (size_t)W * H;
    auto take = [&](size_t b) { char* r = p ? p + o : nullptr; o += align256(b); return r; };
    v.ranges = (uint32_t*)take(8 * (tiles ? tiles : 1));
    v.final_T = (float*)take(4 * (px ? px : 1));
    v.n_contrib = (uint32_t*)take(4 * (px ? px : 1));
    v.bytes = o;
    return v;
}
inline int tile_bits(int W, int H) {
    unsigned tiles = (unsigned)(((W + kTile - 1) / kTile) * ((H + kTile - 1) / kTile));
    int b = 0;
    while ((1u << b) < tiles && b < 31) ++b;
    return b > 0 ? b : 1;
}
inline BinningView carve_binning(void* base, int64_t D, int W, int H) {
    BinningView v;
    char* p = (char*)base;
    size_t o = 0;
    size_t n = (size_t)(D > 0 ? D : 1);
    v.nsort = sort_blocks(n, kSortWavesD);
    v.key_bits = tile_bits(W, H);
    v.passes = (v.key_bits + 7) / 8;
    auto take = [&](size_t b) { char* r = p ? p + o : nullptr; o += align256(b); return r; };
    const unsigned tiles = (unsigned)(((W + kTile - 1) / kTile) * ((H + kTile - 1) / kTile));
    v.key_bytes = tiles <= 65536u ? 2 : 4;
    const int gx = (W + kTile - 1) / kTile, gy = (H + kTile - 1) / kTile;
    v.v2 = binning_v2_ok(gx, gy) ? 1 : 0;
    v.col_rel = nullptr;
    if (v.v2) {
        v.nsort = (int)((n / kEx2Chunk + (size_t)gx + 1 + 3) / 4 * 4);
        v.passes = 1;
        v.key_bytes = 2;
    }
    v.keys[0] = take((size_t)v.key_bytes * n);
    v.keys[1] = take((size_t)v.key_bytes * n);
    v.vals[0] = (uint32_t*)take(4 * n);
    v.vals[1] = (uint32_t*)take(4 * n);
    v.block_hist = (uint32_t*)take(4 * 256 * (size_t)v.nsort);
    v.digit_tot = (uint32_t*)take(4 * 256);
    if (v.v2) v.col_rel = (uint32_t*)take(4 * (size_t)gy * (size_t)(gx + 1));
    v.bytes = o;
    return v;
}

__device__ __forceinline__ float affine3(float m0, float m1, float m2, float m3, float x, float y, float z) {
    return __builtin_fmaf(m2, z, __builtin_fmaf(m1, y, __builtin_fmaf(m0, x, m3)));
}
__device__ __forceinline__ float dot3(float a0, float a1, float a2, float b0, float b1, float b2) {
#pragma clang fp contract(off)
    return __builtin_fmaf(a2, b2, __builtin_fmaf(a1, b1, a0 * b0));
}

__device__ __forceinline__ void tile_rect(float px, float py, int radius, int gx, int gy, int& x0,
                                          int& y0, int& x1, int& y1) {
#pragma clang fp contract(off)
    x0 = min(gx, max(0, (int)((px - (float)radius) / (float)kTile)));
    y0 = min(gy, max(0, (int)((py - (float)radius) / (float)kTile)));
    x1 = min(gx, max(0, (int)((px + (float)radius + (float)(kTile - 1)) / (float)kTile)));
    y1 = min(gy, max(0, (int)((py + (float)radius + (float)(kTile - 1)) / (float)kTile)));
}

__device__ constexpr float SH_C0 = 0.28209479177387814f;
__device__ constexpr float SH_C1 = 0.4886025119029199f;
__device__ constexpr float SH_C2[5] = {1.0925484305920792f, -1.0925484305920792f, 0.31539156525252005f,
                                       -1.0925484305920792f, 0.5462742152960396f};
__device__ constexpr float SH_C3[7] = {-0.5900435899266435f, 2.890611442640554f, -0.4570457994644658f,
                                       0.3731763325901154f,  -0.4570457994644658f, 1.445305721320277f,
                                       -0.5900435899266435f};

__device__ __forceinline__ void sh_basis(int deg, float x, float y, float z, float* b) {
#pragma clang fp contract(off)
    b[0] = SH_C0;
    if (deg > 0) {
        b[1] = -SH_C1 * y;
        b[2] = SH_C1 * z;
        b[3] = -SH_C1 * x;
        if (deg > 1) {
            float xx = x * x, yy = y * y, zz = z * z, xy = x * y, yz = y * z, xz = x * z;
            b[4] = SH_C2[0] * xy;
            b[5] = SH_C2[1] * yz;
            b[6] = SH_C2[2] * (2.0f * zz - xx - yy);
            b[7] = SH_C2[3] * xz;
            b[8] = SH_C2[4] * (xx - yy);
            if (deg > 2) {
                b[9] = SH_C3[0] * y * (3.0f * xx - yy);
                b[10] = SH_C3[1] * xy * z;
                b[11] = SH_C3[2] * y * (4.0f * zz - xx - yy);
                b[12] = SH_C3[3] * z * (2.0f * zz - 3.0f * xx - 3.0f * yy);
                b[13] = SH_C3[4] * x * (4.0f * zz - xx - yy);
                b[14] = SH_C3[5] * z * (xx - yy);
                b[15] = SH_C3[6] * x * (xx - 3.0f * yy);
            }
        }
    }
}

__device__ __forceinline__ void sh_direction(float px, float py, float pz, const float* __restrict__ campos, float& dx, float& dy,
                                             float& dz) {
#pragma clang fp contract(off)
    dx = px - campos[0]; dy = py - campos[1]; dz = pz - campos[2];
    const float len = sqrtf(dot3(dx, dy, dz, dx, dy, dz));
    dx = dx / len; dy = dy / len; dz = dz / len;
}
__device__ __forceinline__ void sh_first(float b0, float c0, float c1, float c2, float& r0, float& r1, float& r2) {
#pragma clang fp contract(off)
    r0 = b0 * c0; r1 = b0 * c1; r2 = b0 * c2;
}
__device__ __forceinline__ void sh_next(float bk, float c0, float c1, float c2, float& r0, float& r1, float& r2) {
    r0 = __builtin_fmaf(bk, c0, r0); r1 = __builtin_fmaf(bk, c1, r1); r2 = __builtin_fmaf(bk, c2, r2);
}
__device__ __forceinline__ void sh_finish(float& r0, float& r1, float& r2, uint32_t& clamp_bits) {
#pragma clang fp contract(off)
    r0 += 0.5f; r1 += 0.5f; r2 += 0.5f;
    clamp_bits = (r0 < 0.0f ? 1u : 0u) | (r1 < 0.0f ? 2u : 0u) | (r2 < 0.0f ? 4u : 0u);
    r0 = fmaxf(r0, 0.0f); r1 = fmaxf(r1, 0.0f); r2 = fmaxf(r2, 0.0f);
}
template <typename Coef>
__device__ __forceinline__ void sh_rgb(int deg, float px, float py, float pz, const float* __restrict__ campos, Coef coef,
                                       float& r0, float& r1, float& r2, uint32_t& clamp_bits) {
    float dx, dy, dz, bs[16];
    sh_direction(px, py, pz, campos, dx, dy, dz);
    sh_basis(deg, dx, dy, dz, bs);
    const int nb = (deg + 1) * (deg + 1);
    sh_first(bs[0], coef(0, 0), coef(0, 1), coef(0, 2), r0, r1, r2);
    for (int k = 1; k < nb; ++k) sh_next(bs[k], coef(k, 0), coef(k, 1), coef(k, 2), r0, r1, r2);
    sh_finish(r0, r1, r2, clamp_bits);
}

template <int DEG>
__device__ __forceinline__ float4 resolve_color_deg(const ColorSource& cs, const float* __restrict__ campos, uint32_t id, float depth,
                                                    float4* rgbd, uint8_t* clamped) {
    constexpr int NB = (DEG + 1) * (DEG + 1), KC = 8;
    const size_t si = (size_t)id;
    const float* row = cs.raw ? cs.shs_rest + si * (size_t)(3 * cs.M - 3) - 3 : cs.shs + si * (size_t)(3 * cs.M);
    float dx, dy, dz, bs[NB > 1 ? NB : 1], r0 = 0.f, r1 = 0.f, r2 = 0.f;
    sh_direction(cs.means3D[3 * si], cs.means3D[3 * si + 1], cs.means3D[3 * si + 2], campos, dx, dy, dz);
    {
        float b16[16];
        sh_basis(DEG, dx, dy, dz, b16);
#pragma unroll
        for (int k = 0; k < NB; ++k) bs[k] = b16[k];
    }
#pragma unroll
    for (int k0 = 0; k0 < NB; k0 += KC) {
        constexpr int kMaxF = 3 * KC;
        const int nk = NB - k0 < KC ? NB - k0 : KC;
        float v[kMaxF];
        if (!cs.raw && cs.vec16) {
#pragma unroll
            for (int q = 0; q < kMaxF / 4; ++q) {
                if (4 * q < 3 * nk) {
                    const float4 t = reinterpret_cast<const float4*>(row + 3 * k0)[q];
                    v[4 * q] = t.x; v[4 * q + 1] = t.y; v[4 * q + 2] = t.z; v[4 * q + 3] = t.w;
                }
            }
        } else {
#pragma unroll
            for (int j = 0; j < kMaxF; ++j)
                if (j < 3 * nk) v[j] = (cs.raw && k0 == 0 && j < 3) ? cs.shs[3 * si + j] : row[3 * k0 + j];
        }
#pragma unroll
        for (int k = 0; k < KC; ++k) {
            if (k < nk) {
                if (k0 + k == 0) sh_first(bs[0], v[0], v[1], v[2], r0, r1, r2);
                else sh_next(bs[k0 + k], v[3 * k], v[3 * k + 1], v[3 * k + 2], r0, r1, r2);
            }
        }
        __builtin_amdgcn_sched_barrier(0);
    }
    uint32_t bits;
    sh_finish(r0, r1, r2, bits);
    const float4 out = make_float4(r0, r1, r2, depth);
    rgbd[si] = out;
    clamped[si] = (uint8_t)bits;
    return out;
}
__device__ __forceinline__ float4 resolve_color(const ColorSource& cs, const float* __restrict__ campos, uint32_t id, float depth,
                                             float4* rgbd, uint8_t* clamped) {
    switch (cs.deg) {
        case 0: return resolve_color_deg<0>(cs, campos, id, depth, rgbd, clamped);
        case 1: return resolve_color_deg<1>(cs, campos, id, depth, rgbd, clamped);
        case 2: return resolve_color_deg<2>(cs, campos, id, depth, rgbd, clamped);
        default: return resolve_color_deg<3>(cs, campos, id, depth, rgbd, clamped);
    }
}
__device__ __forceinline__ float4 resolve_color_small(const ColorSource& cs, const float* __restrict__ campos, uint32_t id,
                                                      float depth, float4* rgbd, uint8_t* clamped) {
    const size_t si = (size_t)id;
    const float* c0p = cs.shs + (cs.raw ? 3 * si : si * (size_t)(3 * cs.M));
    const float* row = cs.raw ? cs.shs_rest + si * (size_t)(3 * cs.M - 3) - 3 : cs.shs + si * (size_t)(3 * cs.M);
    float dx, dy, dz, bs[16], r0, r1, r2;
    sh_direction(cs.means3D[3 * si], cs.means3D[3 * si + 1], cs.means3D[3 * si + 2], campos, dx, dy, dz);
    sh_basis(cs.deg, dx, dy, dz, bs);
    struct F3 { float a, b, c; };
    {
        const F3 t = *reinterpret_cast<const F3*>(c0p);
        sh_first(bs[0], t.a, t.b, t.c, r0, r1, r2);
    }
    auto band = [&](auto first_c, auto last_c) __attribute__((always_inline)) {
        constexpr int kFirst = decltype(first_c)::value, kLast = decltype(last_c)::value;
        F3 t[kLast - kFirst + 1];
#pragma unroll
        for (int k = kFirst; k <= kLast; ++k) t[k - kFirst] = *reinterpret_cast<const F3*>(row + 3 * k);
#pragma unroll
        for (int k = kFirst; k <= kLast; ++k) sh_next(bs[k], t[k - kFirst].a, t[k - kFirst].b, t[k - kFirst].c, r0, r1, r2);
    };
    using std::integral_constant;
    if (cs.deg > 0) {
        band(integral_constant<int, 1>{}, integral_constant<int, 3>{});
        if (cs.deg > 1) {
            band(integral_constant<int, 4>{}, integral_constant<int, 6>{});
            __builtin_amdgcn_sched_barrier(0);
            band(integral_constant<int, 7>{}, integral_constant<int, 8>{});
            if (cs.deg > 2) {
                band(integral_constant<int, 9>{}, integral_constant<int, 12>{});
                __builtin_amdgcn_sched_barrier(0);
                band(integral_constant<int, 13>{}, integral_constant<int, 15>{});
            }
        }
    }
    uint32_t bits;
    sh_finish(r0, r1, r2, bits);
    const float4 out = make_float4(r0, r1, r2, depth);
    rgbd[si] = out;
    clamped[si] = (uint8_t)bits;
    return out;
}
__device__ __forceinline__ bool color_pending(float4 cd) { return cd.x < 0.0f || cd.y < 0.0f || cd.z < 0.0f; }

template <int CTRL, int ROW_MASK>
__device__ __forceinline__ float dpp_add(float v) {
    int t = __builtin_amdgcn_update_dpp(0, __float_as_int(v), CTRL, ROW_MASK, 0xf, true);
    return v + __int_as_float(t);
}
__device__ __forceinline__ float wave_sum_to_lane63(float v) {
    v = dpp_add<0xb1, 0xf>(v);
    v = dpp_add<0x4e, 0xf>(v);
    v = dpp_add<0x114, 0xf>(v);
    v = dpp_add<0x118, 0xf>(v);
    v = dpp_add<0x142, 0xa>(v);
    v = dpp_add<0x143, 0xc>(v);
    return v;
}
__device__ __forceinline__ float row_sum_to_lane15(float v) {
    v = dpp_add<0xb1, 0xf>(v);
    v = dpp_add<0x4e, 0xf>(v);
    v = dpp_add<0x114, 0xf>(v);
    v = dpp_add<0x118, 0xf>(v);
    return v;
}
__device__ __forceinline__ uint32_t wave_sum_u32(uint32_t v) {
    for (int o = 32; o > 0; o >>= 1) v += __shfl_xor(v, o);
    return v;
}

enum Stage { kStPreFwd = 0, kStScan, kStDup, kStSort, kStRanges, kStRenderFwd, kStRenderBwd, kStPreBwd };
void stage_begin(int stage, hipStream_t st);
void stage_end(int stage, hipStream_t st);
struct StageTimer {
    int stage; hipStream_t st;
    StageTimer(int s, hipStream_t q) : stage(s), st(q) { stage_begin(stage, st); }
    ~StageTimer() { stage_end(stage, st); }
};

constexpr int kMaxZero = 10;
struct ZeroRegions {
    float* head[kMaxZero];
    uint4* body[kMaxZero];
    float* tail[kMaxZero];
    uint32_t n_head[kMaxZero], n_body[kMaxZero], n_tail[kMaxZero];
    int n = 0;
    bool overflow = false;
    void add(void* ptr, size_t words) {
        if (!ptr || !words) return;
        if (n >= kMaxZero) { overflow = true; return; }
        float* p = (float*)ptr;
        const size_t mis = ((uintptr_t)p & 15u) / 4u;
        size_t h = mis ? 4 - mis : 0;
        if (h > words) h = words;
        const size_t b = (words - h) / 4, t = words - h - 4 * b;
        head[n] = p; n_head[n] = (uint32_t)h;
        body[n] = (uint4*)(p + h); n_body[n] = (uint32_t)b;
        tail[n] = p + h + 4 * b; n_tail[n] = (uint32_t)t;
        ++n;
    }
};
__device__ __forceinline__ void zero_share(const ZeroRegions& z, int tid, int nthreads) {
    for (int r = 0; r < z.n; ++r) {
        const uint32_t per = (z.n_body[r] + gridDim.x - 1) / gridDim.x;
        const size_t z0 = (size_t)blockIdx.x * per;
        typedef uint32_t zero_u32x4 __attribute__((ext_vector_type(4)));
        const zero_u32x4 zz = {0u, 0u, 0u, 0u};
        for (uint32_t i = tid; i < per && z0 + i < z.n_body[r]; i += nthreads)
            asm volatile("global_store_dwordx4 %0, %1, off sc1" ::"v"(z.body[r] + z0 + i), "v"(zz) : "memory");
        if (blockIdx.x == 0) {
            if (tid < (int)z.n_head[r]) z.head[r][tid] = 0.f;
            if (tid < (int)z.n_tail[r]) z.tail[r][tid] = 0.f;
        }
    }
}
int launch_zero_regions(const ZeroRegions& z, hipStream_t st);

int launch_preprocess_forward(const Frame& f, const float* means3D, const float* shs,
                              const float* colors_precomp, const float* opacities, const float* scales,
                              const float* rotations, const float* cov3D_precomp, GeomView g,
                              int32_t* radii, hipStream_t st);
struct RawBackwardExtra { const float* raw_opacity = nullptr; float* dL_dshs_rest = nullptr; int rows_prezeroed = 0; };
int launch_preprocess_backward_sparse(const Frame& f, const float* means3D, const float* shs, const float* scales,
                                      const float* rotations, const float* cov3D_precomp, GeomView g, const float* grad_rows,
                                      float* dL_dmeans3D, float* dL_dmeans2D, float* dL_dopacity, float* dL_dcolors,
                                      float* dL_dshs, float* dL_dcov3D, float* dL_dscales, float* dL_drots, hipStream_t st,
                                      RawBackwardExtra raw);
int launch_preprocess_backward(const Frame& f, const float* means3D, const float* shs,
                               const float* scales, const float* rotations, const float* cov3D_precomp,
                               const int32_t* radii, GeomView g, const float* grad_rows, float* dL_dmeans3D,
                               float* dL_dmeans2D, float* dL_dopacity, float* dL_dcolors, float* dL_dshs,
                               float* dL_dcov3D, float* dL_dscales, float* dL_drots, hipStream_t st,
                               RawBackwardExtra raw = RawBackwardExtra());
int launch_binning(const Frame& f, GeomView g, const int32_t* radii, BinningView b, ImageView im,
                   int64_t D, hipStream_t st);
int launch_zero_fill(void* p, size_t bytes, hipStream_t st);
int launch_binning2_totals(GeomView g, int P, unsigned long long* totals_host_devptr, hipStream_t st);
int launch_binning2_level1(const Frame& f, GeomView g, hipStream_t st);
int launch_binning2(const Frame& f, GeomView g, BinningView b, ImageView im, int64_t D, int64_t segments, hipStream_t st);
int launch_render_forward(const Frame& f, GeomView g, BinningView b, ImageView im, int64_t D,
                          float* out_color, float* out_depth, hipStream_t st, float* zero_rows = nullptr);
int launch_resolve_colors(const Frame& f, GeomView g, hipStream_t st);
int launch_render_backward(const Frame& f, GeomView g, BinningView b, ImageView im, int64_t D,
                           const float* dL_dpix, float* grad_rows, hipStream_t st, const ZeroRegions* zero = nullptr);
constexpr int kGradRow = 16;
int launch_sh_backward_views(int P, int M, int deg, int n_views, const float* means3D, const float* campos,
                             int64_t campos_stride, const float* gcol, int64_t gcol_stride, float* dL_dshs, hipStream_t st);
int launch_mark_visible(int P, const float* means3D, const float* view, uint8_t* visible, hipStream_t st);
int launch_color_factors(int P, const int32_t* radii, const float* grad_rows, const uint8_t* clamped, float* out, hipStream_t st);

}
```

### multiview_inpaint_amd/csrc/raster_render.hip

```cpp
#include <cstdlib>

#include "raster_common.h"

namespace mvi {

__device__ __forceinline__ unsigned long long ballot64(bool p) { return __builtin_amdgcn_ballot_w64(p); }


__device__ __forceinline__ float active_t2(float4 co) {
    float t2 = 2.0f * __logf(255.0f * co.w);
    return t2 > 0.0f ? t2 * 1.001f + 0.01f : -1.0f;
}

__device__ __forceinline__ bool quad_overlap(float2 c, float4 co, float t2, float qx0, float qy0, float bw = 7.0f,
                                             float bh = 7.0f) {
    const float dxl = qx0 - c.x, dxr = dxl + bw, dyl = qy0 - c.y, dyr = dyl + bh;
    const float px = fminf(fmaxf(0.0f, dxl), dxr), py = fminf(fmaxf(0.0f, dyl), dyr);
    const float dy1 = fminf(fmaxf(-co.y * px * __builtin_amdgcn_rcpf(co.z), dyl), dyr);
    const float dx2 = fminf(fmaxf(-co.y * py * __builtin_amdgcn_rcpf(co.x), dxl), dxr);
    const float f1 = co.x * px * px + 2.0f * co.y * px * dy1 + co.z * dy1 * dy1;
    const float f2 = co.x * dx2 * dx2 + 2.0f * co.y * dx2 * py + co.z * py * py;
    const float f = px == 0.0f ? (py == 0.0f ? 0.0f : f2) : (py == 0.0f ? f1 : fminf(f1, f2));
    return f <= t2;
}

__device__ __forceinline__ int xcd_band_tile(int bid, int tiles) {
    const int q = tiles >> 3, r = tiles & 7, x = bid & 7, i = bid >> 3;
    return x * q + (x < r ? x : r) + i;
}

typedef float f2 __attribute__((ext_vector_type(2)));
__device__ __forceinline__ f2 pk_fma(f2 a, f2 b, f2 c) { return __builtin_elementwise_fma(a, b, c); }
__device__ __forceinline__ f2 splat(float v) { return f2{v, v}; }
constexpr int kB2 = 128;

__device__ __forceinline__ f2 gauss_power(float4 co, float dx, f2 dy) {
#pragma clang fp contract(off)
    const float ax = co.x * dx, bx = co.y * dx;
    const f2 cyy = (co.z * dy) * dy;
    const f2 sq = pk_fma(splat(dx), splat(ax), cyy);
    const f2 bxy = bx * dy;
    return pk_fma(sq, splat(-0.5f), -bxy);
}

__device__ __forceinline__ float gauss_power1(float4 co, float dx, float dy) {
#pragma clang fp contract(off)
    const float ax = co.x * dx, bx = co.y * dx;
    const float cyy = (co.z * dy) * dy;
    const float sq = __builtin_fmaf(dx, ax, cyy);
    const float bxy = bx * dy;
    return __builtin_fmaf(sq, -0.5f, -bxy);
}

__global__ __launch_bounds__(kBlock) void render_forward_kernel(
    Frame f, const uint32_t* __restrict__ ranges, const uint32_t* __restrict__ point_list,
    const float2* __restrict__ xy, float4* rgbd, const float4* __restrict__ conic_opacity,
    float* __restrict__ final_T, uint32_t* __restrict__ n_contrib, float* __restrict__ out_color,
    float* __restrict__ out_depth, ZeroRegions zero, const ColorSource* __restrict__ color_src, uint8_t* clamped) {
    __shared__ float2 s_xy[kBlock];
    __shared__ float s_t2[kBlock];
    __shared__ float4 s_co[kBlock];
    __shared__ float4 s_cd[kBlock];
    __shared__ float4 w_s[4][3][64];
    const int tid = threadIdx.x, wave = tid >> 6, lane = tid & 63;
    zero_share(zero, tid, kBlock);
    const int tile = xcd_band_tile(blockIdx.x, f.gx * f.gy);
    const int tile_y = tile / f.gx, tile_x = tile - tile_y * f.gx;
    const int qx0 = tile_x * kTile + 8 * (wave & 1), qy0 = tile_y * kTile + 8 * (wave >> 1);
    const int pxi = qx0 + (lane & 7), pyi = qy0 + (lane >> 3);
    const bool inside = pxi < f.W && pyi < f.H;
    const float pfx = (float)pxi, pfy = (float)pyi;
    const uint32_t r0 = ranges[2 * tile], r1 = ranges[2 * tile + 1];
    int todo = (int)(r1 - r0);
    const int rounds = (todo + kBlock - 1) / kBlock;

    float T = inside ? 1.0f : 0.0f;
    float T_out = 1.0f, C2 = 0.f, Dp = kDepthSentinel, Tc = 1.0f;
    f2 C01 = {0.f, 0.f};
    uint32_t last = 0;

    const ColorSource cs = *color_src;
    float2 n_xy = make_float2(0.f, 0.f);
    float4 n_co = make_float4(0.f, 0.f, 0.f, 0.f), n_cd = n_co;
    uint32_t n_id = 0;
    auto fetch = [&](int r) {
        const uint32_t q = r0 + (uint32_t)(r * kBlock + tid);
        if (q < r1) {
            n_id = point_list[q];
            n_xy = xy[n_id]; n_co = conic_opacity[n_id]; n_cd = rgbd[n_id];
        }
    };
    if (rounds > 0) fetch(0);
    for (int r = 0; r < rounds; ++r, todo -= kBlock) {
        if (__syncthreads_count(T <= 0.0f) == kBlock) break;
        if (cs.deferred && tid < todo && color_pending(n_cd)) n_cd = resolve_color_small(cs, f.campos, n_id, n_cd.w, rgbd, clamped);
        s_xy[tid] = n_xy;
        s_co[tid] = n_co;
        s_t2[tid] = active_t2(n_co);
        s_cd[tid] = n_cd;
        __syncthreads();
        if (r + 1 < rounds) fetch(r + 1);
        const int n = todo < kBlock ? todo : kBlock;
        for (int c = 0; c < n; c += 64) {
            if (ballot64(T > 0.0f) == 0ull) break;
            const int e = c + lane;
            const bool keep = e < n && quad_overlap(s_xy[e], s_co[e], s_t2[e], (float)qx0, (float)qy0);
            const unsigned long long mask = ballot64(keep);
            if (mask == 0ull) continue;
            if (keep) {
                const int pos = __builtin_amdgcn_mbcnt_hi((uint32_t)(mask >> 32), __builtin_amdgcn_mbcnt_lo((uint32_t)mask, 0u));
                const float2 q = s_xy[e];
                w_s[wave][0][pos] = make_float4(q.x, q.y, __uint_as_float((uint32_t)(r * kBlock + e + 1)), 0.f);
                w_s[wave][1][pos] = s_co[e];
                w_s[wave][2][pos] = s_cd[e];
            }
            const int cnt = __popcll(mask);
            float4 a = w_s[wave][0][0], co = w_s[wave][1][0], cd = w_s[wave][2][0];
            for (int k = 0; k < cnt; ++k) {
                const int kn = k + 1 < 64 ? k + 1 : 63;
                const float4* nx = &w_s[wave][0][kn];
                const float4 an = nx[0], con = nx[64], cdn = nx[128];
                float dx = a.x - pfx, dy = a.y - pfy;
                float power = gauss_power1(co, dx, dy);
                float alpha = fminf(kAlphaMax, co.w * __expf(power));
                alpha = power <= 0.0f ? alpha : 0.0f;
                const float test_T = T * (1.0f - alpha);
                const bool valid = alpha >= kAlphaMin;
                const bool contrib = valid && test_T >= kTEps;
                const float w = contrib ? alpha * T : 0.0f;
                C01 = pk_fma(f2{cd.x, cd.y}, splat(w), C01);
                C2 = __builtin_fmaf(cd.z, w, C2);
                const bool above = contrib && T > 0.5f;
                Dp = above ? cd.w : Dp;
                Tc = above ? test_T : Tc;
                T_out = contrib ? test_T : T_out;
                last = contrib ? __float_as_uint(a.z) : last;
                T = contrib ? test_T : (valid ? 0.0f : T);
                a = an; co = con; cd = cdn;
            }
        }
    }
    if (inside) {
        size_t pix = (size_t)pyi * f.W + pxi, hw = (size_t)f.H * f.W;
        final_T[pix] = T_out;
        n_contrib[pix] = last;
        out_color[pix] = C01.x + T_out * f.bg[0];
        out_color[hw + pix] = C01.y + T_out * f.bg[1];
        out_color[2 * hw + pix] = C2 + T_out * f.bg[2];
        out_depth[pix] = Tc < 0.5f ? Dp : kDepthSentinel;
    }
}

constexpr int kFrontTiles = 4;
constexpr int kFrontMax = 1024;
__global__ __launch_bounds__(kBlock) void mark_front_kernel(int tiles, const uint32_t* __restrict__ ranges,
                                                            const uint32_t* __restrict__ point_list, uint8_t* __restrict__ front,
                                                            int n_front, const ColorSource* __restrict__ color_src, int gx,
                                                            int every) {
    if (!color_src->deferred) return;
    const int tid = threadIdx.x;
    const int sx = (gx + every - 1) / every;
#pragma unroll
    for (int t = 0; t < kFrontTiles; ++t) {
        const int j = blockIdx.x * kFrontTiles + t;
        const int tile = every == 1 ? j : (j / sx) * every * gx + (j % sx) * every;
        if (tile >= tiles) break;
        const uint32_t r0 = ranges[2 * tile], r1 = ranges[2 * tile + 1];
        const uint32_t n = min(r1 - r0, (uint32_t)n_front);
        for (uint32_t e = tid; e < n; e += kBlock) front[point_list[r0 + e]] = 1;
    }
}
constexpr int kMarkedPer = 4;
__global__ __launch_bounds__(kBlock) void resolve_marked_kernel(Frame f, GeomView g) {
    const ColorSource cs = *g.color_src;
    if (!cs.deferred) return;
    __shared__ uint32_t s_id[kBlock * kMarkedPer];
    __shared__ uint32_t s_n;
    const int tid = threadIdx.x;
    if (tid == 0) s_n = 0;
    __syncthreads();
    const int i0 = (blockIdx.x * kBlock + tid) * kMarkedPer;
    if (i0 < f.P) {
        const uint32_t w = *reinterpret_cast<const uint32_t*>(g.front + i0);
#pragma unroll
        for (int k = 0; k < kMarkedPer; ++k)
            if (((w >> (8 * k)) & 0xFFu) && i0 + k < f.P) s_id[atomicAdd(&s_n, 1u)] = (uint32_t)(i0 + k);
    }
    __syncthreads();
    const uint32_t total = s_n;
    for (uint32_t i = tid; i < total; i += kBlock) {
        const uint32_t id = s_id[i];
        const float4 cd = g.rgbd[id];
        if (color_pending(cd)) resolve_color(cs, f.campos, id, cd.w, g.rgbd, g.clamped);
    }
}

int launch_zero_fill(void* p, size_t bytes, hipStream_t st);
int launch_render_forward(const Frame& f, GeomView g, BinningView b, ImageView im, int64_t D,
                          float* out_color, float* out_depth, hipStream_t st, float* zero_rows) {
    ZeroRegions z;
    if (zero_rows) {
        z.add(zero_rows, (size_t)f.P * kGradRow);
        z.add(g.touched, ((size_t)f.P + 15) / 16 * 4);
        z.add(g.touched_count, 1);
    }
    if (f.W <= 0 || f.H <= 0) return launch_zero_regions(z, st);
    const uint32_t* plist = b.vals[b.passes & 1];
    const unsigned blocks = (unsigned)(f.gx * f.gy);
    if (f.defer_colors && D > 0) {
        static const int n_front = [] { const char* e = getenv("MVI_RASTER_FRONT_ENTRIES"); const int v = e ? atoi(e) : kBlock;
                                        return v < 0 ? 0 : (v > kFrontMax ? kFrontMax : v); }();
        static const int every = [] { const char* e = getenv("MVI_RASTER_FRONT_EVERY"); const int v = e ? atoi(e) : 2; return v < 1 ? 1 : v; }();
        if (n_front > 0) {
            const unsigned sampled = (unsigned)(((f.gx + every - 1) / every) * ((f.gy + every - 1) / every));
            hipLaunchKernelGGL(mark_front_kernel, dim3((sampled + kFrontTiles - 1) / kFrontTiles), dim3(kBlock), 0, st, (int)blocks,
                               im.ranges, plist, g.front, n_front, g.color_src, f.gx, every);
            hipLaunchKernelGGL(resolve_marked_kernel, dim3((f.P + kBlock * kMarkedPer - 1) / (kBlock * kMarkedPer)), dim3(kBlock), 0, st,
                               f, g);
        }
    }
    hipLaunchKernelGGL(render_forward_kernel, dim3(blocks), dim3(kBlock), 0, st, f, im.ranges, plist, g.xy,
                       g.rgbd, g.conic_opacity, im.final_T, im.n_contrib, out_color, out_depth, z, g.color_src, g.clamped);
    return hipGetLastError() == hipSuccess ? 0 : MVI_EHIP;
}

__global__ __launch_bounds__(256) void zero_regions_kernel(ZeroRegions z) { zero_share(z, threadIdx.x, 256); }
int launch_zero_regions(const ZeroRegions& z, hipStream_t st) {
    if (z.n == 0) return 0;
    hipLaunchKernelGGL(zero_regions_kernel, dim3(2048), dim3(256), 0, st, z);
    return hipGetLastError() == hipSuccess ? 0 : MVI_EHIP;
}

constexpr int kRow = 16;
#ifndef MVI_RB_SLAB
#define MVI_RB_SLAB 3
#endif
constexpr int kSlabG = MVI_RB_SLAB;
constexpr int kSlabStride = 20;


#define MVI_DPP1 " quad_perm:[1,0,3,2] row_mask:0xf bank_mask:0xf bound_ctrl:1\n\t"
#define MVI_DPP2 " quad_perm:[2,3,0,1] row_mask:0xf bank_mask:0xf bound_ctrl:1\n\t"
__device__ __forceinline__ void quad_sum9(float& a, float& b, float& c, float& d, float& e, float& f, float& g, float& h,
                                          float& i) {
    asm("s_nop 1\n\t"
        "v_add_f32_dpp %0, %0, %0" MVI_DPP1 "v_add_f32_dpp %1, %1, %1" MVI_DPP1 "v_add_f32_dpp %2, %2, %2" MVI_DPP1
        "v_add_f32_dpp %3, %3, %3" MVI_DPP1 "v_add_f32_dpp %4, %4, %4" MVI_DPP1 "v_add_f32_dpp %5, %5, %5" MVI_DPP1
        "v_add_f32_dpp %6, %6, %6" MVI_DPP1 "v_add_f32_dpp %7, %7, %7" MVI_DPP1 "v_add_f32_dpp %8, %8, %8" MVI_DPP1
        "v_add_f32_dpp %0, %0, %0" MVI_DPP2 "v_add_f32_dpp %1, %1, %1" MVI_DPP2 "v_add_f32_dpp %2, %2, %2" MVI_DPP2
        "v_add_f32_dpp %3, %3, %3" MVI_DPP2 "v_add_f32_dpp %4, %4, %4" MVI_DPP2 "v_add_f32_dpp %5, %5, %5" MVI_DPP2
        "v_add_f32_dpp %6, %6, %6" MVI_DPP2 "v_add_f32_dpp %7, %7, %7" MVI_DPP2 "v_add_f32_dpp %8, %8, %8" MVI_DPP2
        : "+v"(a), "+v"(b), "+v"(c), "+v"(d), "+v"(e), "+v"(f), "+v"(g), "+v"(h), "+v"(i));
}
#undef MVI_DPP1
#undef MVI_DPP2

#ifndef MVI_RB_WAVES
#define MVI_RB_WAVES 5
#endif
__global__ __launch_bounds__(kB2) __attribute__((amdgpu_waves_per_eu(MVI_RB_WAVES, MVI_RB_WAVES))) void render_backward_kernel(
    Frame f, const uint32_t* __restrict__ ranges, const uint32_t* __restrict__ point_list,
    const float2* __restrict__ xy, const float4* __restrict__ rgbd, const float4* __restrict__ conic_opacity,
    const float* __restrict__ final_T, const uint32_t* __restrict__ n_contrib,
    const float* __restrict__ dL_dpix, float* __restrict__ grad_rows, uint8_t* __restrict__ touched, ZeroRegions zero) {
#pragma clang fp contract(off)
    zero_share(zero, threadIdx.x, kB2);
    __shared__ uint32_t s_id[kB2];
    __shared__ float2 s_xy[kB2];
    __shared__ float s_t2[kB2];
    __shared__ float4 s_co[kB2];
    __shared__ float4 s_rgb[kB2];
    __shared__ float s_acc[kB2][9];
    __shared__ __attribute__((aligned(16))) float s_slab[2][kSlabG * 9][kSlabStride];
    __shared__ int s_slot[2][8];
    __shared__ uint32_t s_blast[2];
    const int tid = threadIdx.x, wave = tid >> 6, lane = tid & 63;
    const int tile = xcd_band_tile(blockIdx.x, f.gx * f.gy);
    const int tile_y = tile / f.gx, tile_x = tile - tile_y * f.gx;
    const int hx0 = tile_x * kTile, hy0 = tile_y * kTile + 8 * wave;
    const int pxi = hx0 + (lane & 15), py0 = hy0 + 2 * (lane >> 4), py1 = py0 + 1;
    const bool in0 = pxi < f.W && py0 < f.H, in1 = pxi < f.W && py1 < f.H;
    const float pfx = (float)pxi;
    const f2 pfy = {(float)py0, (float)py1};
    const uint32_t r0 = ranges[2 * tile];
    const size_t hw = (size_t)f.H * f.W, pix0 = (size_t)py0 * f.W + pxi, pix1 = pix0 + f.W;

    const f2 T_final = {in0 ? final_T[pix0] : 0.0f, in1 ? final_T[pix1] : 0.0f};
    f2 T = T_final;
    const uint32_t last0 = in0 ? n_contrib[pix0] : 0u, last1 = in1 ? n_contrib[pix1] : 0u;
    f2 A_dot = {0.f, 0.f};
    f2 dp0 = {0.f, 0.f}, dp1 = {0.f, 0.f}, dp2 = {0.f, 0.f};
    if (in0) { dp0.x = dL_dpix[pix0]; dp1.x = dL_dpix[hw + pix0]; dp2.x = dL_dpix[2 * hw + pix0]; }
    if (in1) { dp0.y = dL_dpix[pix1]; dp1.y = dL_dpix[hw + pix1]; dp2.y = dL_dpix[2 * hw + pix1]; }
    const f2 bg_dot = f.bg[0] * dp0 + f.bg[1] * dp1 + f.bg[2] * dp2;
    const f2 bg_term = -T_final * bg_dot;
    uint32_t wave_last = max(last0, last1);
    for (int o = 32; o > 0; o >>= 1) wave_last = max(wave_last, (uint32_t)__shfl_xor((int)wave_last, o));
    if (lane == 0) s_blast[wave] = wave_last;
    __syncthreads();
    const int total = (int)max(s_blast[0], s_blast[1]);
    const int rounds = (total + kB2 - 1) / kB2;
    const int my_slot = (lane * 57) >> 9, my_mom = lane - 9 * my_slot;
    float (*slab)[kSlabStride] = s_slab[wave];
    auto drain = [&](int parked) {
        if (lane < 9 * parked) {
            const float4* row = reinterpret_cast<const float4*>(slab[lane]);
            float4 a = row[0], b = row[1], c = row[2], d = row[3];
            float sum = ((a.x + a.y) + (a.z + a.w)) + ((b.x + b.y) + (b.z + b.w)) + ((c.x + c.y) + (c.z + c.w)) +
                        ((d.x + d.y) + (d.z + d.w));
            atomicAdd(&s_acc[0][0] + (__mul24(s_slot[wave][my_slot], 9) + my_mom), sum);
        }
    };

    uint32_t n_id = 0;
    float2 n_xy = make_float2(0.f, 0.f);
    float4 n_co = make_float4(0.f, 0.f, 0.f, 0.f), n_cd = n_co;
    auto fetch = [&](int r) {
        const int hi_ = total - r * kB2;
        if (tid < hi_) {
            n_id = point_list[r0 + (uint32_t)(hi_ - 1 - tid)];
            n_xy = xy[n_id]; n_co = conic_opacity[n_id]; n_cd = rgbd[n_id];
        }
    };
    if (rounds > 0) fetch(0);
    for (int r = 0; r < rounds; ++r) {
        const int hi = total - r * kB2;
        const int n = hi < kB2 ? hi : kB2;
        __syncthreads();
        s_id[tid] = n_id;
        s_xy[tid] = n_xy;
        s_co[tid] = n_co;
        s_t2[tid] = active_t2(n_co);
        s_rgb[tid] = n_cd;
#pragma unroll
        for (int c = 0; c < 9; ++c) s_acc[tid][c] = 0.0f;
        __syncthreads();
        if (r + 1 < rounds) fetch(r + 1);
        int parked = 0;
        for (int c = 0; c < n; c += 64) {
            const int e = c + lane;
            const bool keep = e < n && (uint32_t)(hi - 1 - e) < wave_last &&
                              quad_overlap(s_xy[e], s_co[e], s_t2[e], (float)hx0, (float)hy0, 15.0f, 7.0f);
            unsigned long long mask = ballot64(keep);
            if (mask == 0ull) continue;
            int j = c + __builtin_ctzll(mask);
            auto entry = [&](const int jc, const float2 p, const float4 co, const float4 col, float2& nx_p, float4& nx_co,
                             float4& nx_col, int& jn) -> bool {
                mask &= mask - 1;
                const bool more = mask != 0ull;
                jn = more ? c + __builtin_ctzll(mask) : jc;
                nx_p = s_xy[jn];
                nx_co = s_co[jn];
                nx_col = s_rgb[jn];
                const uint32_t pos = (uint32_t)(hi - 1 - jc);
                const float dx = p.x - pfx;
                const f2 dy = splat(p.y) - pfy;
                const f2 power = gauss_power(co, dx, dy);
                const f2 G = {__expf(power.x), __expf(power.y)};
                const f2 oG = co.w * G;
                const f2 alpha = __builtin_elementwise_min(splat(kAlphaMax), oG);
                const bool act0 = pos < last0 && power.x <= 0.0f && alpha.x >= kAlphaMin;
                const bool act1 = pos < last1 && power.y <= 0.0f && alpha.y >= kAlphaMin;
                const f2 am = {act0 ? alpha.x : 0.0f, act1 ? alpha.y : 0.0f};
                const f2 gm = {act0 ? oG.x : 0.0f, act1 ? oG.y : 0.0f};
                const unsigned long long any_active = ballot64((__float_as_uint(am.x) | __float_as_uint(am.y)) != 0u);
                const f2 om = splat(1.0f) - am;
                const f2 inv = {__builtin_amdgcn_rcpf(om.x), __builtin_amdgcn_rcpf(om.y)};
                const f2 Tn = T * inv;
                const f2 c_dot = pk_fma(splat(col.z), dp2, pk_fma(splat(col.y), dp1, col.x * dp0));
                const f2 dL_dalpha = pk_fma(c_dot - A_dot, Tn, bg_term * inv);
                const f2 dch = am * Tn, mw = gm * dL_dalpha;
                T = Tn;
                A_dot = pk_fma(am, c_dot, om * A_dot);
                if (any_active != 0ull) {
                    const f2 vr = dch * dp0, vg = dch * dp1, vb = dch * dp2;
                    const f2 vx = mw * dx, vy = mw * dy;
                    const f2 vxx = vx * dx, vxy = vx * dy, vyy = vy * dy;
                    float m_w = mw.x + mw.y, m_x = vx.x + vx.y, m_y = vy.x + vy.y, m_xx = vxx.x + vxx.y,
                          m_xy = vxy.x + vxy.y, m_yy = vyy.x + vyy.y, m_r = vr.x + vr.y, m_g = vg.x + vg.y, m_b = vb.x + vb.y;
                    quad_sum9(m_w, m_x, m_y, m_xx, m_xy, m_yy, m_r, m_g, m_b);
                    const int pk = __builtin_amdgcn_readfirstlane(parked);
                    if ((lane & 3) == 3) {
                        float* colp = &slab[0][0] + (pk * (9 * kSlabStride) + (lane >> 2));
                        colp[0 * kSlabStride] = m_w;  colp[1 * kSlabStride] = m_x;  colp[2 * kSlabStride] = m_y;
                        colp[3 * kSlabStride] = m_xx; colp[4 * kSlabStride] = m_xy; colp[5 * kSlabStride] = m_yy;
                        colp[6 * kSlabStride] = m_r;  colp[7 * kSlabStride] = m_g;  colp[8 * kSlabStride] = m_b;
                    }
                    if (lane == 0) s_slot[wave][pk] = jc;
                    parked = pk + 1;
                    if (parked == kSlabG) { drain(kSlabG); parked = 0; }
                }
                return more;
            };
            float2 pA = s_xy[j], pB;
            float4 coA = s_co[j], coB, colA = s_rgb[j], colB;
            int jB = j;
            while (true) {
                if (!entry(j, pA, coA, colA, pB, coB, colB, jB)) break;
                if (!entry(jB, pB, coB, colB, pA, coA, colA, j)) break;
            }
        }
        if (parked) drain(parked);
        __syncthreads();
        {
            const int e1 = wave * 64 + lane;
            if (e1 < n) {
                float* a = s_acc[e1];
                const float a0 = a[0], a1 = a[1], a2 = a[2], a3 = a[3], a4 = a[4], a5 = a[5], a6 = a[6], a7 = a[7], a8 = a[8];
                const bool any = (((__float_as_uint(a0) | __float_as_uint(a1) | __float_as_uint(a2)) |
                                   (__float_as_uint(a3) | __float_as_uint(a4) | __float_as_uint(a5)) |
                                   (__float_as_uint(a6) | __float_as_uint(a7) | __float_as_uint(a8))) & 0x7FFFFFFFu) != 0u;
                if (any) {
                    const float4 co = s_co[e1];
                    a[0] = -0.5f * (float)f.W * (co.x * a1 + co.y * a2);
                    a[1] = -0.5f * (float)f.H * (co.z * a2 + co.y * a1);
                    a[2] = -0.5f * a3;
                    a[3] = -a4;
                    a[4] = -0.5f * a5;
                    a[5] = a0 / co.w;
                } else {
                    s_id[e1] = 0xFFFFFFFFu;
                }
            }
            asm volatile("s_waitcnt lgkmcnt(0)" ::: "memory");
            __builtin_amdgcn_wave_barrier();
            const int comp = lane & 15;
#pragma unroll 4
            for (int it = 0; it < 16; ++it) {
                const int e = wave * 64 + it * 4 + (lane >> 4);
                const uint32_t id = e < n ? s_id[e] : 0xFFFFFFFFu;
                if (id == 0xFFFFFFFFu || comp >= 9) continue;
                atomicAdd(&grad_rows[(size_t)id * kRow + comp], s_acc[e][comp]);
                if (comp == 0) touched[id] = 1;
            }
        }
    }
}

int launch_render_backward(const Frame& f, GeomView g, BinningView b, ImageView im, int64_t D,
                           const float* dL_dpix, float* grad_rows, hipStream_t st, const ZeroRegions* zero) {
    ZeroRegions z;
    if (zero) z = *zero;
    if (f.W <= 0 || f.H <= 0 || D <= 0) return launch_zero_regions(z, st);
    const uint32_t* plist = b.vals[b.passes & 1];
    hipLaunchKernelGGL(render_backward_kernel, dim3(f.gx * f.gy), dim3(kB2), 0, st, f, im.ranges, plist, g.xy,
                       g.rgbd, g.conic_opacity, im.final_T, im.n_contrib, dL_dpix, grad_rows, g.touched, z);
    return hipGetLastError() == hipSuccess ? 0 : MVI_EHIP;
}

}
```

Measured before the change: 2201 Mpix/s.

## Make binning expand kernels persistent with prefetch and fold front marking

Turns row_count and expand_scatter into persistent kernels sized to resident occupancy. Each block walks chunks in serpentine order and prefetches the next chunk's inputs while processing the current one. The per-bin global scan is hoisted out of the loop, and front-entry marking for deferred colours moves into the pass-2 expand kernel, so the separate mark_front kernel can be skipped. This cuts launch and tail cost and overlaps loads with compute, at the price of higher register pressure and extra complexity.

Result: no change. 2217 Mpix/s, median of 6 (+0.7%).

```diff
diff --git a/include/mvi_raster.h b/include/mvi_raster.h
--- a/include/mvi_raster.h
+++ b/include/mvi_raster.h
@@ -117,6 +117,7 @@
     const uint32_t* n_contrib;
     int32_t tile_id_bytes;
     const uint8_t* grad_support;
+    const uint8_t* front;
 } mvi_raster_views;
 int mvi_raster_get_views(int32_t P, int64_t num_rendered, int32_t image_width, int32_t image_height,
                          const void* geom, const void* binning, const void* image,
@@ -129,6 +130,7 @@
 const char* mvi_raster_stage_name(int stage);
 
 int mvi_raster_color_mode(int deferred);
+int mvi_raster_front_config(int fold, int entries, int every);
 int mvi_raster_resolve_colors(const mvi_raster_settings* s, int32_t P, void* geom, size_t geom_bytes, void* stream);
 
 int mvi_raster_binning_version(int version);
diff --git a/multiview_inpaint_amd/_lib.py b/multiview_inpaint_amd/_lib.py
--- a/multiview_inpaint_amd/_lib.py
+++ b/multiview_inpaint_amd/_lib.py
@@ -24,7 +24,8 @@
     _fields_ = [(n, C.c_void_p) for n in (
         "depths", "means2D", "cov3D_a", "cov3D_b", "conic_opacity", "rgbd", "tiles_touched", "clamped",
         "tile_ids_sorted", "point_list", "ranges", "final_T", "n_contrib")] + [("tile_id_bytes", C.c_int32),
-                                                                                   ("grad_support", C.c_void_p)]
+                                                                                   ("grad_support", C.c_void_p),
+                                                                                   ("front", C.c_void_p)]
 
 
 class AdamGroup(C.Structure):
@@ -121,6 +122,8 @@
     L.mvi_raster_backward_mode.argtypes = [C.c_int]
     L.mvi_raster_color_mode.restype = C.c_int
     L.mvi_raster_color_mode.argtypes = [C.c_int]
+    L.mvi_raster_front_config.restype = C.c_int
+    L.mvi_raster_front_config.argtypes = [C.c_int, C.c_int, C.c_int]
     L.mvi_raster_resolve_colors.restype = C.c_int
     L.mvi_raster_resolve_colors.argtypes = [C.POINTER(RasterSettings), i32, vp, sz, vp]
     L.mvi_raster_dev_stamps.restype = C.c_int
diff --git a/multiview_inpaint_amd/csrc/raster_api.hip b/multiview_inpaint_amd/csrc/raster_api.hip
--- a/multiview_inpaint_amd/csrc/raster_api.hip
+++ b/multiview_inpaint_amd/csrc/raster_api.hip
@@ -130,6 +130,7 @@
     if (deferred == 0 || deferred == 1) g_defer_colors = deferred;
     return old;
 }
+int mvi_raster_front_config(int fold, int entries, int every) { return mvi::set_front_config(fold, entries, every); }
 int mvi_raster_resolve_colors(const mvi_raster_settings* s, int32_t P, void* geom, size_t geom_bytes, void* stream) {
     mvi::Frame f;
     if (int rc = make_frame(s, P, 0, f)) return rc;
@@ -254,6 +255,7 @@
     if (D > 0 && geom_bytes < g.bytes) return fail(MVI_ENOMEM, "geom scratch too small%s", "");
     hipStream_t st = (hipStream_t)stream;
     const int64_t segments = recall_segments(geom, P);
+    b.front_marked = (f.bin_v2 && f.defer_colors && mvi::front_fold_enabled() && mvi::front_entries() > 0) ? 1 : 0;
     if (f.bin_v2 ? mvi::launch_binning2(f, g, b, im, D, segments, st) : mvi::launch_binning(f, g, radii, b, im, D, st))
         return hip_fail("binning", hipGetLastError());
     {
@@ -532,6 +534,7 @@
         out->conic_opacity = reinterpret_cast<const float*>(g.conic_opacity); out->rgbd = reinterpret_cast<const float*>(g.rgbd);
         out->tiles_touched = g.tiles_touched; out->clamped = g.clamped;
         out->grad_support = g.touched;
+        out->front = g.front;
     }
     if (binning) {
         mvi::BinningView b = mvi::carve_binning(const_cast<void*>(binning), D, W, H);
diff --git a/multiview_inpaint_amd/csrc/raster_binning2.hip b/multiview_inpaint_amd/csrc/raster_binning2.hip
--- a/multiview_inpaint_amd/csrc/raster_binning2.hip
+++ b/multiview_inpaint_amd/csrc/raster_binning2.hip
@@ -1,3 +1,4 @@
+#include <atomic>
 #include <cstdlib>
 
 #include "raster_common.h"
@@ -331,22 +332,26 @@
     build_chunk_table(tot, gx, tid, chunk_first, col_start, s_w4);
 }
 struct Chunk { int x; uint32_t seg0, seg1; bool first; };
-__device__ __forceinline__ bool load_chunk(const uint32_t* __restrict__ chunk_first, const uint32_t* __restrict__ col_start,
-                                           int gx, int tid, uint32_t* s_first, uint32_t* s_col, Chunk& ck) {
+__device__ __forceinline__ void load_chunk_table(const uint32_t* __restrict__ chunk_first, const uint32_t* __restrict__ col_start,
+                                                 int gx, int tid, uint32_t* s_first, uint32_t* s_col) {
     if (tid <= gx) { s_first[tid] = chunk_first[tid]; s_col[tid] = col_start[tid]; }
-    __syncthreads();
-    const uint32_t c = blockIdx.x;
-    if (c >= s_first[gx]) return false;
+}
+__device__ __forceinline__ Chunk locate_chunk(uint32_t c, int gx, const uint32_t* s_first, const uint32_t* s_col) {
     int lo = 0, hi = gx - 1;
     while (lo < hi) {
         const int mid = (lo + hi + 1) >> 1;
         if (s_first[mid] <= c) lo = mid; else hi = mid - 1;
     }
+    Chunk ck;
     ck.x = lo;
     ck.first = c == s_first[lo];
     ck.seg0 = s_col[lo] + (c - s_first[lo]) * (uint32_t)kEx2Chunk;
     ck.seg1 = min(ck.seg0 + (uint32_t)kEx2Chunk, s_col[lo + 1]);
-    return true;
+    return ck;
+}
+
+__device__ __forceinline__ uint32_t chunk_of_round(uint32_t round, uint32_t grid) {
+    return round * grid + ((round & 1u) ? grid - 1u - blockIdx.x : blockIdx.x);
 }
 
 __global__ __launch_bounds__(kExThreads) void row_count_kernel(int gx, int gy, const uint32_t* __restrict__ chunk_first,
@@ -356,23 +361,41 @@
     __shared__ uint32_t s_first[257], s_col[257], s_w4[4];
     __shared__ uint32_t s_d[257];
     const int tid = threadIdx.x;
-    if (tid <= 256) s_d[tid] = 0;
-    Chunk ck;
-    if (!load_chunk(chunk_first, col_start, gx, tid, s_first, s_col, ck)) return;
-#pragma unroll
-    for (int k = 0; k < kEx2Items; ++k) {
-        const uint32_t i = ck.seg0 + (uint32_t)(k * kExThreads + tid);
-        if (i < ck.seg1) {
-            const uint32_t yh = seg_yh[i];
-            const uint32_t y0 = yh & 255u, h = (yh >> 8) + 1u;
-            atomicAdd(&s_d[y0], 1u);
-            atomicSub(&s_d[y0 + h], 1u);
-        }
-    }
-    __syncthreads();
-    const uint32_t v = tid < 256 ? s_d[tid] : 0u;
-    const uint32_t ex = block_excl_scan256(v, tid, s_w4, nullptr);
-    if (tid < gy) row_table[(size_t)tid * stride + blockIdx.x] = ex + v;
+    load_chunk_table(chunk_first, col_start, gx, tid, s_first, s_col);
+    __syncthreads();
+    const uint32_t nchunks = s_first[gx], grid = gridDim.x;
+    uint32_t chunk = blockIdx.x, round = 0;
+    if (chunk >= nchunks) return;
+    auto request = [&](uint32_t c, uint32_t (&yh)[kEx2Items]) {
+        const Chunk ck = locate_chunk(c, gx, s_first, s_col);
+#pragma unroll
+        for (int k = 0; k < kEx2Items; ++k) {
+            const uint32_t i = ck.seg0 + (uint32_t)(k * kExThreads + tid);
+            yh[k] = i < ck.seg1 ? (uint32_t)seg_yh[i] : 0xFFFF0000u;
+        }
+    };
+    uint32_t yh[kEx2Items];
+    request(chunk, yh);
+    for (;;) {
+        if (tid <= 256) s_d[tid] = 0;
+        __syncthreads();
+#pragma unroll
+        for (int k = 0; k < kEx2Items; ++k) {
+            if (yh[k] != 0xFFFF0000u) {
+                const uint32_t y0 = yh[k] & 255u, h = (yh[k] >> 8) + 1u;
+                atomicAdd(&s_d[y0], 1u);
+                atomicSub(&s_d[y0 + h], 1u);
+            }
+        }
+        const uint32_t next = chunk_of_round(++round, grid);
+        if (next < nchunks) request(next, yh);
+        __syncthreads();
+        const uint32_t v = tid < 256 ? s_d[tid] : 0u;
+        const uint32_t ex = block_excl_scan256(v, tid, s_w4, nullptr);
+        if (tid < gy) row_table[(size_t)tid * stride + chunk] = ex + v;
+        if (next >= nchunks) break;
+        chunk = next;
+    }
 }
 
 __global__ __launch_bounds__(1024) void row_scan_kernel(int gx, const uint32_t* __restrict__ chunk_first,
@@ -414,6 +437,7 @@
 
 struct ExpandArgs {
     int n_items;
+    int nchunks;
     int nbins;
     int gx;
     const uint32_t* order;
@@ -424,6 +448,9 @@
     const uint16_t* seg_yh_in;
     const uint32_t* col_rel;
     uint32_t* ranges;
+    uint8_t* front;
+    const ColorSource* color_src;
+    int front_entries, front_every;
     const uint32_t* table;
     const uint32_t* tot;
     int stride;
@@ -433,27 +460,26 @@
 };
 static unsigned long long* g_dev_stamps[2] = {nullptr, nullptr};
 void set_dev_stamps(int pass, void* buf) { if (pass == 1 || pass == 2) g_dev_stamps[pass - 1] = (unsigned long long*)buf; }
-#define MVI_STAMP(i) do { if (A.stamps && tid == 0) A.stamps[(size_t)blk * 8 + (i)] = __builtin_amdgcn_s_memtime(); } while (0)
-
-__device__ __forceinline__ void block_excl_scan512x2(uint32_t a, uint32_t b, int tid, uint32_t (*s_w)[8], uint32_t& ea,
-                                                     uint32_t& ta, uint32_t& eb) {
+#define MVI_STAMP(i) do { if (A.stamps && tid == 0) A.stamps[(size_t)chunk * 8 + (i)] = __builtin_amdgcn_s_memtime(); } while (0)
+
+__device__ __forceinline__ void block_excl_scan512(uint32_t a, int tid, uint32_t* s_w, uint32_t& ea, uint32_t& ta) {
     const int lane = tid & 63, wave = tid >> 6;
-    uint32_t ia = a, ib = b;
+    uint32_t ia = a;
 #pragma unroll
     for (int o = 1; o < 64; o <<= 1) {
-        const uint32_t x = __shfl_up(ia, o), y = __shfl_up(ib, o);
-        if (lane >= o) { ia += x; ib += y; }
-    }
-    if (lane == 63) { s_w[0][wave] = ia; s_w[1][wave] = ib; }
-    __syncthreads();
-    uint32_t oa = 0, ob = 0, t = 0;
+        const uint32_t x = __shfl_up(ia, o);
+        if (lane >= o) ia += x;
+    }
+    if (lane == 63) s_w[wave] = ia;
+    __syncthreads();
+    uint32_t oa = 0, t = 0;
 #pragma unroll
     for (int w = 0; w < 8; ++w) {
-        const uint32_t x = s_w[0][w], y = s_w[1][w];
-        if (w < wave) { oa += x; ob += y; }
+        const uint32_t x = s_w[w];
+        if (w < wave) oa += x;
         t += x;
     }
-    ea = oa + ia - a; eb = ob + ib - b; ta = t;
+    ea = oa + ia - a; ta = t;
 }
 
 template <int PASS, int NB, int ITEMS, int CAP>
@@ -464,156 +490,238 @@
     constexpr int kStride = NB + 1;
     static_assert(kCap >= 64 * NB, "a round of 64 items (<= 64 * NB entries) always fits the image");
     static_assert(kRounds >= 16, "worker parts <= rounds");
-    static_assert(kExThreads == 512, "block_excl_scan512x2");
+    static_assert(kExThreads == 512, "block_excl_scan512");
     __shared__ alignas(16) unsigned long long s_mask[kRounds * kStride + 1];
     __shared__ uint32_t s_pay[kChunk];
     __shared__ uint16_t s_aux[PASS == 1 ? kChunk : 1];
     __shared__ uint32_t s_img[kCap];
-    __shared__ uint32_t s_lstart[NB + 1], s_delta[NB];
+    __shared__ uint32_t s_lstart[NB + 1];
+    __shared__ uint2 s_out[NB];
     __shared__ uint32_t s_rtot[kRounds];
-    __shared__ uint32_t s_w[2][8];
-    uint32_t* const s_first = s_img;
-    uint32_t* const s_col = s_img + 257;
+    __shared__ uint32_t s_w[8];
+    __shared__ uint32_t s_first[PASS == 2 ? 257 : 1], s_col[PASS == 2 ? 257 : 1];
     const int tid = threadIdx.x, lane = tid & 63, wave = tid >> 6;
-    const uint32_t blk = blockIdx.x;
-
-    uint32_t item0 = 0, item1 = 0;
-    Chunk ck{0, 0u, 0u, false};
-    if (PASS == 1) {
-        item0 = blk * (uint32_t)kChunk;
-        item1 = min(item0 + (uint32_t)kChunk, (uint32_t)A.n_items);
-    } else {
-        if (!load_chunk(A.chunk_first, A.col_start, A.gx, tid, s_first, s_col, ck)) return;
-        item0 = ck.seg0; item1 = ck.seg1;
-    }
-    MVI_STAMP(0);
-    uint32_t ia[ITEMS], in_[ITEMS];
-#pragma unroll
-    for (int k = 0; k < ITEMS; ++k) {
-        const int li = (wave * ITEMS + k) * 64 + lane;
-        const uint32_t i = item0 + (uint32_t)li;
-        ia[k] = 0; in_[k] = 0;
-        uint32_t pay = 0, aux = 0;
-        if (i < item1) {
-            if (PASS == 1) {
-                const uint2 rc = A.rect_sorted[i];
-                const uint32_t w = rc.y & 0xFFFFu, h = rc.y >> 16;
-                if (w * h) {
-                    ia[k] = rc.x & 0xFFFFu; in_[k] = w;
-                    pay = A.order[i];
-                    aux = (rc.x >> 16) | ((h - 1u) << 8);
-                }
-            } else {
-                const uint32_t yh = A.seg_yh_in[i];
-                ia[k] = yh & 255u; in_[k] = (yh >> 8) + 1u;
-                pay = A.seg_idx_in[i];
-            }
-        }
-        s_pay[li] = pay;
-        if (PASS == 1) s_aux[li] = (uint16_t)aux;
-    }
+    const uint32_t grid = gridDim.x;
+
+    auto clear_masks = [&]() {
+        uint4* m4 = reinterpret_cast<uint4*>(&s_mask[0]);
+        for (int i = tid; i < (kRounds * kStride + 1) / 2; i += kExThreads) m4[i] = make_uint4(0u, 0u, 0u, 0u);
+        if (tid < kRounds) s_rtot[tid] = 0;
+    };
+    clear_masks();
+    if (PASS == 2) load_chunk_table(A.chunk_first, A.col_start, A.gx, tid, s_first, s_col);
+    __syncthreads();
+    const uint32_t nchunks = PASS == 1 ? (uint32_t)A.nchunks : s_first[A.gx];
+    uint32_t chunk = blockIdx.x, round = 0;
+    if (chunk >= nchunks) return;
+
     const int nb = A.nbins;
     const int parts = min(kExThreads / nb, 16);
     const bool worker = tid < parts * nb;
     const int b = worker ? tid / parts : 0, q = worker ? tid % parts : 0;
     const int r_lo = worker ? q * kRounds / parts : 0, r_hi = worker ? (q + 1) * kRounds / parts : 0;
     const bool bin_head = worker && q == 0;
-    const uint32_t bin_tot = bin_head ? A.tot[b] : 0u;
-    const uint32_t bin_off = bin_head ? A.table[(size_t)b * A.stride + blk] : 0u;
-    {
-        uint4* m4 = reinterpret_cast<uint4*>(&s_mask[0]);
-        for (int i = tid; i < (kRounds * kStride + 1) / 2; i += kExThreads) m4[i] = make_uint4(0u, 0u, 0u, 0u);
-        if (tid < kRounds) s_rtot[tid] = 0;
-    }
-    __syncthreads();
-    MVI_STAMP(1);
-
-    const unsigned long long bit = 1ull << lane;
-#pragma unroll
-    for (int k = 0; k < ITEMS; ++k) {
-        unsigned long long* row = s_mask + (wave * ITEMS + k) * kStride;
-        for (uint32_t i = 0; i < in_[k]; ++i) atomicOr(&row[ia[k] + i], bit);
-    }
-    __syncthreads();
-    MVI_STAMP(2);
-
     const unsigned long long* mcol = s_mask + b;
-    uint32_t my_base = 0, my_goff = 0;
-
-    int g0 = 0, g1 = kRounds;
-    bool first = true, have_rtot = false;
+    bool mark_row = false;
+    if (PASS == 2 && A.front) mark_row = A.color_src->deferred != 0 && bin_head && b % A.front_every == 0;
+
+    struct Ahead {
+        Chunk ck;
+        uint32_t item0, item1;
+        uint2 rc[PASS == 1 ? ITEMS : 1];
+        uint32_t yh[PASS == 2 ? ITEMS : 1];
+        uint32_t pay[ITEMS];
+        uint32_t bin_off, rel0, rel1;
+    };
+    auto request = [&](uint32_t c, Ahead& n) {
+        if (PASS == 1) {
+            n.ck = Chunk{0, 0u, 0u, false};
+            n.item0 = c * (uint32_t)kChunk;
+            n.item1 = min(n.item0 + (uint32_t)kChunk, (uint32_t)A.n_items);
+        } else {
+            n.ck = locate_chunk(c, A.gx, s_first, s_col);
+            n.item0 = n.ck.seg0; n.item1 = n.ck.seg1;
+        }
+#pragma unroll
+        for (int k = 0; k < ITEMS; ++k) {
+            const uint32_t i = n.item0 + (uint32_t)((wave * ITEMS + k) * 64 + lane);
+            const bool valid = i < n.item1;
+            if (PASS == 1) {
+                n.rc[k] = valid ? A.rect_sorted[i] : make_uint2(0u, 0u);
+                n.pay[k] = valid ? A.order[i] : 0u;
+            } else {
+                n.yh[k] = valid ? (uint32_t)A.seg_yh_in[i] : 0xFFFF0000u;
+                n.pay[k] = valid ? A.seg_idx_in[i] : 0u;
+            }
+        }
+        n.bin_off = bin_head ? A.table[(size_t)b * A.stride + c] : 0u;
+        n.rel0 = 0u; n.rel1 = 0u;
+        if (PASS == 2 && bin_head) {
+            const uint32_t* cr = A.col_rel + (size_t)b * (A.gx + 1) + n.ck.x;
+            n.rel0 = cr[0];
+            if (n.ck.first) n.rel1 = cr[1];
+        }
+    };
+    Ahead nx;
+    request(chunk, nx);
+    uint32_t bin_start, all_entries;
+    block_excl_scan512(bin_head ? A.tot[b] : 0u, tid, s_w, bin_start, all_entries);
+
     for (;;) {
-        uint32_t cnt = 0;
-        for (int r = max(r_lo, g0); r < min(r_hi, g1); ++r) cnt += (uint32_t)__popcll(mcol[r * kStride]);
-        uint32_t pos0, total, bin_start;
-        block_excl_scan512x2(cnt, first ? bin_tot : 0u, tid, s_w, pos0, total, bin_start);
-        if (first) {
-            first = false;
-            my_base = bin_start + bin_off;
-            if (PASS == 2 && ck.first && bin_head) {
-                const uint32_t* cr = A.col_rel + (size_t)b * (A.gx + 1);
-                const uint32_t c = cr[ck.x + 1] - cr[ck.x];
-                uint2* rg = reinterpret_cast<uint2*>(A.ranges) + ((size_t)b * A.gx + ck.x);
-                *rg = c ? make_uint2(my_base, my_base + c) : make_uint2(0u, 0u);
-            }
-            if (total == 0) return;
-        }
-        MVI_STAMP(3);
-        if (total > (uint32_t)kCap) {
-            if (!have_rtot) {
-                have_rtot = true;
-                for (int r = r_lo; r < r_hi; ++r) {
-                    const uint32_t c = (uint32_t)__popcll(mcol[r * kStride]);
-                    if (c) atomicAdd(&s_rtot[r], c);
+        MVI_STAMP(0);
+        const Chunk ck = nx.ck;
+        const uint32_t bin_off = nx.bin_off, rel0 = nx.rel0, rel1 = nx.rel1;
+        uint32_t ia[ITEMS], in_[ITEMS];
+#pragma unroll
+        for (int k = 0; k < ITEMS; ++k) {
+            const int li = (wave * ITEMS + k) * 64 + lane;
+            ia[k] = 0; in_[k] = 0;
+            uint32_t pay = 0, aux = 0;
+            if (PASS == 1) {
+                const uint2 rc = nx.rc[k];
+                const uint32_t w = rc.y & 0xFFFFu, h = rc.y >> 16;
+                if (w * h) {
+                    ia[k] = rc.x & 0xFFFFu; in_[k] = w;
+                    pay = nx.pay[k];
+                    aux = (rc.x >> 16) | ((h - 1u) << 8);
                 }
+            } else if (nx.yh[k] != 0xFFFF0000u) {
+                ia[k] = nx.yh[k] & 255u; in_[k] = (nx.yh[k] >> 8) + 1u;
+                pay = nx.pay[k];
+            }
+            s_pay[li] = pay;
+            if (PASS == 1) s_aux[li] = (uint16_t)aux;
+        }
+        MVI_STAMP(1);
+
+        const unsigned long long bit = 1ull << lane;
+#pragma unroll
+        for (int k = 0; k < ITEMS; ++k) {
+            unsigned long long* row = s_mask + (wave * ITEMS + k) * kStride;
+            for (uint32_t i = 0; i < in_[k]; ++i) atomicOr(&row[ia[k] + i], bit);
+        }
+        const uint32_t next = chunk_of_round(++round, grid);
+        if (next < nchunks) request(next, nx);
+        __syncthreads();
+        MVI_STAMP(2);
+
+        const uint32_t my_base = bin_start + bin_off;
+        uint32_t my_goff = 0;
+        uint32_t front_lim = 0;
+        if (PASS == 2 && mark_row && ck.x % A.front_every == 0) {
+            const unsigned long long lim = (unsigned long long)bin_start + rel0 + (unsigned long long)A.front_entries;
+            front_lim = lim > 0xFFFFFFFFull ? 0xFFFFFFFFu : (uint32_t)lim;
+        }
+        if (PASS == 2 && ck.first && bin_head) {
+            const uint32_t c = rel1 - rel0;
+            uint2* rg = reinterpret_cast<uint2*>(A.ranges) + ((size_t)b * A.gx + ck.x);
+            *rg = c ? make_uint2(my_base, my_base + c) : make_uint2(0u, 0u);
+        }
+
+        int g0 = 0, g1 = kRounds;
+        bool first = true, have_rtot = false;
+        for (;;) {
+            uint32_t cnt = 0;
+            for (int r = max(r_lo, g0); r < min(r_hi, g1); ++r) cnt += (uint32_t)__popcll(mcol[r * kStride]);
+            uint32_t pos0, total;
+            block_excl_scan512(cnt, tid, s_w, pos0, total);
+            if (first) {
+                first = false;
+                if (total == 0) break;
+            }
+            MVI_STAMP(3);
+            if (total > (uint32_t)kCap) {
+                if (!have_rtot) {
+                    have_rtot = true;
+                    for (int r = r_lo; r < r_hi; ++r) {
+                        const uint32_t c = (uint32_t)__popcll(mcol[r * kStride]);
+                        if (c) atomicAdd(&s_rtot[r], c);
+                    }
+                }
+                __syncthreads();
+                uint32_t acc = 0;
+                g1 = g0;
+                while (g1 < kRounds && acc + s_rtot[g1] <= (uint32_t)kCap) { acc += s_rtot[g1]; ++g1; }
+                continue;
+            }
+            if (bin_head) {
+                s_lstart[b] = pos0;
+                s_out[b] = make_uint2(my_base + my_goff - pos0, front_lim);
+            }
+            if (tid == 0) s_lstart[nb] = total;
+            MVI_STAMP(4);
+            if (cnt) {
+                uint32_t pos = pos0;
+                const uint32_t hi = (uint32_t)b << 16;
+                for (int r = max(r_lo, g0); r < min(r_hi, g1); ++r) {
+                    const unsigned long long m = mcol[r * kStride];
+                    uint32_t m0 = (uint32_t)m, m1 = (uint32_t)(m >> 32);
+                    const uint32_t item_hi = hi | (uint32_t)(r * 64);
+                    while (m0) {
+                        const uint32_t l = (uint32_t)__builtin_ctz(m0);
+                        m0 &= m0 - 1u;
+                        s_img[pos++] = item_hi | l;
+                    }
+                    while (m1) {
+                        const uint32_t l = (uint32_t)__builtin_ctz(m1);
+                        m1 &= m1 - 1u;
+                        s_img[pos++] = item_hi | 32u | l;
+                    }
+                }
             }
             __syncthreads();
-            uint32_t acc = 0;
-            g1 = g0;
-            while (g1 < kRounds && acc + s_rtot[g1] <= (uint32_t)kCap) { acc += s_rtot[g1]; ++g1; }
-            continue;
-        }
-        if (bin_head) {
-            s_lstart[b] = pos0;
-            s_delta[b] = my_base + my_goff - pos0;
-        }
-        if (tid == 0) s_lstart[nb] = total;
-        MVI_STAMP(4);
-        if (cnt) {
-            uint32_t pos = pos0;
-            const uint32_t hi = (uint32_t)b << 16;
-            for (int r = max(r_lo, g0); r < min(r_hi, g1); ++r) {
-                const unsigned long long m = mcol[r * kStride];
-                uint32_t m0 = (uint32_t)m, m1 = (uint32_t)(m >> 32);
-                const uint32_t item_hi = hi | (uint32_t)(r * 64);
-                while (m0) {
-                    const uint32_t l = (uint32_t)__builtin_ctz(m0);
-                    m0 &= m0 - 1u;
-                    s_img[pos++] = item_hi | l;
+            MVI_STAMP(5);
+            const bool last_group = g1 >= kRounds;
+            if (last_group) clear_masks();
+            for (uint32_t p = tid; p < total; p += kExThreads) {
+                const uint32_t e = s_img[p];
+                const uint32_t eb = e >> 16, item = e & 0xFFFFu;
+                const uint2 o = s_out[eb];
+                const uint32_t dst = p + o.x;
+                const uint32_t pay = s_pay[item];
+                A.out_idx[dst] = pay;
+                if (PASS == 1) A.out_aux[dst] = s_aux[item];
+                else {
+                    A.out_aux[dst] = (uint16_t)(eb * (uint32_t)A.gx + (uint32_t)ck.x);
+                    if (dst < o.y) A.front[pay] = 1;
                 }
-                while (m1) {
-                    const uint32_t l = (uint32_t)__builtin_ctz(m1);
-                    m1 &= m1 - 1u;
-                    s_img[pos++] = item_hi | 32u | l;
-                }
-            }
-        }
-        __syncthreads();
-        MVI_STAMP(5);
-        for (uint32_t p = tid; p < total; p += kExThreads) {
-            const uint32_t e = s_img[p];
-            const uint32_t eb = e >> 16, item = e & 0xFFFFu;
-            const uint32_t dst = p + s_delta[eb];
-            A.out_idx[dst] = s_pay[item];
-            if (PASS == 1) A.out_aux[dst] = s_aux[item];
-            else A.out_aux[dst] = (uint16_t)(eb * (uint32_t)A.gx + (uint32_t)ck.x);
-        }
-        MVI_STAMP(6);
-        if (g1 >= kRounds) break;
-        if (bin_head) my_goff += s_lstart[b + 1] - pos0;
-        __syncthreads();
-        g0 = g1; g1 = kRounds;
-    }
+            }
+            MVI_STAMP(6);
+            if (last_group) break;
+            if (bin_head) my_goff += s_lstart[b + 1] - pos0;
+            __syncthreads();
+            g0 = g1; g1 = kRounds;
+        }
+        if (next >= nchunks) break;
+        __syncthreads();
+        chunk = next;
+    }
+}
+
+template <auto Kernel>
+static int resident_blocks(int& blocks) {
+    constexpr int kMaxDevices = 64;
+    static std::atomic<int> cache[kMaxDevices];
+    int device = -1;
+    if (hipGetDevice(&device) != hipSuccess || device < 0 || device >= kMaxDevices) return MVI_EHIP;
+    int v = cache[device].load(std::memory_order_relaxed);
+    if (v <= 0) {
+        int per_cu = 0, cus = 0;
+        if (hipOccupancyMaxActiveBlocksPerMultiprocessor(&per_cu, Kernel, kExThreads, 0) != hipSuccess) return MVI_EHIP;
+        if (hipDeviceGetAttribute(&cus, hipDeviceAttributeMultiprocessorCount, device) != hipSuccess) return MVI_EHIP;
+        if (per_cu <= 0 || cus <= 0) return MVI_EHIP;
+        v = per_cu * cus;
+        cache[device].store(v, std::memory_order_relaxed);
+    }
+    blocks = v;
+    return 0;
+}
+template <auto Kernel, typename... Args>
+static int launch_persistent(int chunks, hipStream_t st, Args... args) {
+    int grid = 0;
+    if (int rc = resident_blocks<Kernel>(grid)) return rc;
+    hipLaunchKernelGGL(Kernel, dim3(min(grid, chunks)), dim3(kExThreads), 0, st, args...);
+    return 0;
 }
 
 int launch_binning2_level1(const Frame& f, GeomView g, hipStream_t st) {
@@ -642,16 +750,16 @@
     if (D <= 0 || f.P <= 0) return launch_zero_fill(im.ranges, 8 * tiles, st);
     const bool wide = f.gx > 128 || f.gy > 128;
     ExpandArgs a1{};
-    a1.n_items = f.P; a1.nbins = f.gx; a1.gx = f.gx;
+    a1.n_items = f.P; a1.nchunks = g.nblk1; a1.nbins = f.gx; a1.gx = f.gx;
     a1.order = g.dvals[0]; a1.rect_sorted = g.rect_sorted;
     a1.table = g.col_table; a1.tot = g.col_tot; a1.stride = g.nblk1;
     a1.out_idx = b.vals[0]; a1.out_aux = (uint16_t*)b.keys[0];
     a1.stamps = g_dev_stamps[0];
     {
         StageTimer tm(kStDup, st);
-        if (wide)
-            hipLaunchKernelGGL((expand_scatter_kernel<1, 256, kExItems, 64 * 256>), dim3(g.nblk1), dim3(kExThreads), 0, st, a1);
-        else hipLaunchKernelGGL((expand_scatter_kernel<1, 128, kExItems, 64 * 128>), dim3(g.nblk1), dim3(kExThreads), 0, st, a1);
+        if (int rc = wide ? launch_persistent<expand_scatter_kernel<1, 256, kExItems, 64 * 256>>(g.nblk1, st, a1)
+                          : launch_persistent<expand_scatter_kernel<1, 128, kExItems, 64 * 128>>(g.nblk1, st, a1))
+            return rc;
     }
     int nchunk = b.nsort;
     if (segments > 0 && segments <= D) nchunk = (int)min((int64_t)b.nsort, segments / kEx2Chunk + f.gx + 1);
@@ -660,12 +768,18 @@
     a2.chunk_first = g.chunk_first; a2.col_start = g.col_start;
     a2.seg_idx_in = b.vals[0]; a2.seg_yh_in = (const uint16_t*)b.keys[0];
     a2.col_rel = b.col_rel; a2.ranges = im.ranges;
+    if (b.front_marked) {
+        a2.front = g.front; a2.color_src = g.color_src;
+        a2.front_entries = front_entries(); a2.front_every = front_every();
+    }
     a2.table = b.block_hist; a2.tot = b.digit_tot; a2.stride = b.nsort;
     a2.out_idx = b.vals[1]; a2.out_aux = (uint16_t*)b.keys[1];
     a2.stamps = g_dev_stamps[1];
     StageTimer tm(kStSort, st);
-    hipLaunchKernelGGL(row_count_kernel, dim3(nchunk), dim3(kExThreads), 0, st, f.gx, f.gy, g.chunk_first, g.col_start,
-                       (const uint16_t*)b.keys[0], b.block_hist, b.nsort);
+    if (int rc = launch_persistent<row_count_kernel>(nchunk, st, f.gx, f.gy, (const uint32_t*)g.chunk_first,
+                                                     (const uint32_t*)g.col_start, (const uint16_t*)b.keys[0], b.block_hist,
+                                                     b.nsort))
+        return rc;
     hipLaunchKernelGGL(row_scan_kernel, dim3(f.gy), dim3(1024), 0, st, f.gx, g.chunk_first, b.block_hist, b.nsort,
                        b.digit_tot, b.col_rel);
     if (f.gy <= kEx2SmallNB)
diff --git a/multiview_inpaint_amd/csrc/raster_common.h b/multiview_inpaint_amd/csrc/raster_common.h
--- a/multiview_inpaint_amd/csrc/raster_common.h
+++ b/multiview_inpaint_amd/csrc/raster_common.h
@@ -58,6 +58,10 @@
 void set_dev_stamps(int pass, void* buf);
 int set_binning_version(int v);
 inline bool binning_v2_ok(int gx, int gy) { return gx <= 256 && gy <= 256 && binning_v2_enabled(); }
+int front_entries();
+int front_every();
+bool front_fold_enabled();
+int set_front_config(int fold, int entries, int every);
 
 struct ColorSource {
     const float* means3D;
@@ -122,6 +126,7 @@
     int key_bits;
     int v2;
     uint32_t* col_rel;
+    int front_marked;
     size_t bytes;
 };
 
@@ -206,6 +211,7 @@
     const int gx = (W + kTile - 1) / kTile, gy = (H + kTile - 1) / kTile;
     v.v2 = binning_v2_ok(gx, gy) ? 1 : 0;
     v.col_rel = nullptr;
+    v.front_marked = 0;
     if (v.v2) {
         v.nsort = (int)((n / kEx2Chunk + (size_t)gx + 1 + 3) / 4 * 4);
         v.passes = 1;
diff --git a/multiview_inpaint_amd/csrc/raster_render.hip b/multiview_inpaint_amd/csrc/raster_render.hip
--- a/multiview_inpaint_amd/csrc/raster_render.hip
+++ b/multiview_inpaint_amd/csrc/raster_render.hip
@@ -153,6 +153,20 @@
 
 constexpr int kFrontTiles = 4;
 constexpr int kFrontMax = 1024;
+static int g_front_entries = [] { const char* e = getenv("MVI_RASTER_FRONT_ENTRIES"); const int v = e ? atoi(e) : kBlock;
+                                  return v < 0 ? 0 : (v > kFrontMax ? kFrontMax : v); }();
+static int g_front_every = [] { const char* e = getenv("MVI_RASTER_FRONT_EVERY"); const int v = e ? atoi(e) : 2; return v < 1 ? 1 : v; }();
+static int g_front_fold = [] { const char* e = getenv("MVI_RASTER_FRONT_KERNEL"); return (e && e[0] == '1') ? 0 : 1; }();
+int front_entries() { return g_front_entries; }
+int front_every() { return g_front_every; }
+bool front_fold_enabled() { return g_front_fold != 0; }
+int set_front_config(int fold, int entries, int every) {
+    const int old = g_front_fold;
+    if (fold == 0 || fold == 1) g_front_fold = fold;
+    if (entries >= 0) g_front_entries = entries > kFrontMax ? kFrontMax : entries;
+    if (every >= 1) g_front_every = every;
+    return old;
+}
 __global__ __launch_bounds__(kBlock) void mark_front_kernel(int tiles, const uint32_t* __restrict__ ranges,
                                                             const uint32_t* __restrict__ point_list, uint8_t* __restrict__ front,
                                                             int n_front, const ColorSource* __restrict__ color_src, int gx,
@@ -208,13 +222,12 @@
     const uint32_t* plist = b.vals[b.passes & 1];
     const unsigned blocks = (unsigned)(f.gx * f.gy);
     if (f.defer_colors && D > 0) {
-        static const int n_front = [] { const char* e = getenv("MVI_RASTER_FRONT_ENTRIES"); const int v = e ? atoi(e) : kBlock;
-                                        return v < 0 ? 0 : (v > kFrontMax ? kFrontMax : v); }();
-        static const int every = [] { const char* e = getenv("MVI_RASTER_FRONT_EVERY"); const int v = e ? atoi(e) : 2; return v < 1 ? 1 : v; }();
+        const int n_front = front_entries(), every = front_every();
         if (n_front > 0) {
             const unsigned sampled = (unsigned)(((f.gx + every - 1) / every) * ((f.gy + every - 1) / every));
-            hipLaunchKernelGGL(mark_front_kernel, dim3((sampled + kFrontTiles - 1) / kFrontTiles), dim3(kBlock), 0, st, (int)blocks,
-                               im.ranges, plist, g.front, n_front, g.color_src, f.gx, every);
+            if (!b.front_marked)
+                hipLaunchKernelGGL(mark_front_kernel, dim3((sampled + kFrontTiles - 1) / kFrontTiles), dim3(kBlock), 0, st, (int)blocks,
+                                   im.ranges, plist, g.front, n_front, g.color_src, f.gx, every);
             hipLaunchKernelGGL(resolve_marked_kernel, dim3((f.P + kBlock * kMarkedPer - 1) / (kBlock * kMarkedPer)), dim3(kBlock), 0, st,
                                f, g);
         }
```
